# bacpop/sparrowhawk

Measured on AMD Instinct MI355X. Metric: Gbases/s assembled, k=31 150bp reads, higher is better.
Workload: dtype u64

## Files before the change

include/shk.h:

```cpp
#ifndef SHK_H
#define SHK_H

#include <stddef.h>
#include <stdint.h>

#ifdef __cplusplus
extern "C" {
#endif

#define SHK_OK 0
#define SHK_E_PARAM  (-1)
#define SHK_E_STATE  (-2)
#define SHK_E_PARSE  (-3)
#define SHK_E_OOM    (-4)
#define SHK_E_DEVICE (-5)
#define SHK_E_INTERNAL (-6)

#define SHK_HISTO_BINS 500
#define SHK_K_MIN 15
#define SHK_K_MAX 255

typedef struct shk_handle shk_handle;

typedef void (*shk_progress_cb)(const char *state, void *user);
// ... 66 lines not shown
void shk_packed_free(shk_packed *p);

uint32_t shk_key_words(shk_handle *h);
uint64_t shk_total_instances(shk_handle *h);
uint64_t shk_n_distinct(shk_handle *h);
int shk_get_distinct(shk_handle *h, uint64_t *keys, uint32_t *counts, uint64_t cap);
uint64_t shk_n_solid(shk_handle *h);
int shk_get_solid(shk_handle *h, uint64_t *keys, uint32_t *counts, uint64_t cap);
int shk_get_histo(shk_handle *h, uint64_t *histo500);
uint32_t shk_used_min_count(shk_handle *h);
int shk_get_adjacency(shk_handle *h, uint8_t *adj_initial, uint8_t *adj_final, uint8_t *alive,
                      uint64_t cap);
const char *shk_get_timings(shk_handle *h);
uint64_t shk_peak_device_bytes(shk_handle *h);
void shk_host_mem_counter(const int64_t *deltas, size_t n, uint64_t *peak, uint64_t *current);

int shk_host_canonical(const char *seq, uint32_t k, uint64_t *out_words , int *orient);
uint64_t shk_host_nthash(const char *seq, uint32_t k);
int shk_host_fit(const uint64_t *histo500, uint32_t *used_min_count);
char *shk_host_assembly_json(const char *seqs, const uint64_t *offsets, const uint64_t *kc, uint64_t n_contigs, uint32_t k);
char *shk_host_assembly_json_arriving(const char *seqs, const uint64_t *offsets, const uint64_t *kc, uint64_t n_contigs, uint32_t k,
                                      uint64_t piece_bytes, uint32_t delay_us);
void shk_host_free(void *p);
int shk_host_gunzip(const uint8_t *gz, size_t n, uint8_t **out, size_t *out_n, uint64_t *mt_members, double *reader_seconds);
int shk_device_gunzip(const uint8_t *gz, size_t n, uint8_t **out, size_t *out_n, const char **why, double *ms_total);
char *shk_host_unitig_assemble(uint32_t k, uint64_t n_recs, const uint64_t *first, const uint64_t *last, const uint64_t *len,
                               const uint64_t *kc, const uint8_t *circ, const uint64_t *min_key, const uint8_t *min_o,
                               const uint64_t *min_pos, int tips, int bubbles);
char *shk_device_unitig_assemble(uint32_t k, uint64_t n_recs, const uint64_t *first, const uint64_t *last, const uint64_t *len,
                                 const uint64_t *kc, const uint8_t *circ, const uint64_t *min_key, const uint8_t *min_o,
                                 const uint64_t *min_pos, int tips, int bubbles);

void shk_release_cached_memory(void);

int shk_measure_stream_read(size_t bytes, int iters, double *gbs);

const char *shk_version(void);

#ifdef __cplusplus
}
#endif
#endif
```

sparrowhawk_amd/_lib.py:

```python
import ctypes as C
import os

_HERE = os.path.dirname(os.path.abspath(__file__))
LIB_PATH = os.path.join(_HERE, "libshk_hip.so")

PROGRESS_CB = C.CFUNCTYPE(None, C.c_char_p, C.c_void_p)


class ShkPacked(C.Structure):
    _fields_ = [("bases", C.POINTER(C.c_uint32)), ("seg_off", C.POINTER(C.c_uint32)),
                ("n_seg", C.c_uint64), ("n_bases", C.c_uint64), ("n_reads", C.c_uint64),
                ("n_input_bases", C.c_uint64)]


_u64, _u32, _vp, _cp, _int, _sz = C.c_uint64, C.c_uint32, C.c_void_p, C.c_char_p, C.c_int, C.c_size_t
SIGNATURES = {
    "shk_new": (_vp, [_u32, _int, _u32, _u32, _u64, _int, _int, _int, _int]),
    "shk_new_error": (_int, []),
    "shk_new_error_message": (_cp, []),
    "shk_free": (None, [_vp]),
    "shk_last_error": (_cp, [_vp]),
    "shk_set_progress_cb": (None, [_vp, PROGRESS_CB, _vp]),
    "shk_preprocess": (_int, [_vp, _cp, _sz, _cp, _sz]),
    "shk_push_reads": (_int, [_vp, _cp, _sz]),
# ... 16 lines not shown
    "shk_comm_world": (_int, [_vp]),
    "shk_comm_free": (None, [_vp]),
    "shk_shard_preprocess": (_int, [_vp, _vp, _vp, _vp, _u64, _u64, _u64, _u32]),
    "shk_plan_exchange": (_int, [_vp, _u32, _u32, _u32, _vp, _vp, _vp, _vp, _vp]),
    "shk_choose_partitions": (_u32, [_u64, _u32, _u32]),
    "shk_plan_bgzf_windows": (C.c_int64, [_vp, _u64, _u64, _vp, _u64]),
    "shk_host_last_record_start": (_u64, [_cp, _sz]),
    "shk_device_last_record_start": (_int, [_cp, _sz, C.POINTER(_u64)]),
    "shk_pack_fastq": (_int, [_cp, _sz, _u32, _u32, C.POINTER(ShkPacked), C.POINTER(_cp)]),
    "shk_packed_free": (None, [C.POINTER(ShkPacked)]),
    "shk_key_words": (_u32, [_vp]),
    "shk_total_instances": (_u64, [_vp]),
    "shk_n_distinct": (_u64, [_vp]),
    "shk_get_distinct": (_int, [_vp, _vp, _vp, _u64]),
    "shk_n_solid": (_u64, [_vp]),
    "shk_get_solid": (_int, [_vp, _vp, _vp, _u64]),
    "shk_get_histo": (_int, [_vp, _vp]),
    "shk_used_min_count": (_u32, [_vp]),
    "shk_get_adjacency": (_int, [_vp, _vp, _vp, _vp, _u64]),
    "shk_get_timings": (_cp, [_vp]),
    "shk_peak_device_bytes": (_u64, [_vp]),
    "shk_host_mem_counter": (None, [_vp, _sz, C.POINTER(_u64), C.POINTER(_u64)]),
    "shk_host_canonical": (_int, [_cp, _u32, _vp, C.POINTER(_int)]),
    "shk_host_nthash": (_u64, [_cp, _u32]),
    "shk_host_fit": (_int, [_vp, C.POINTER(_u32)]),
    "shk_host_assembly_json": (_vp, [_cp, _vp, _vp, _u64, _u32]),
    "shk_host_assembly_json_arriving": (_vp, [_cp, _vp, _vp, _u64, _u32, _u64, _u32]),
    "shk_host_free": (None, [_vp]),
    "shk_host_gunzip": (_int, [_cp, _sz, C.POINTER(_vp), C.POINTER(_sz), C.POINTER(_u64), C.POINTER(C.c_double)]),
    "shk_device_gunzip": (_int, [_cp, _sz, C.POINTER(_vp), C.POINTER(_sz), C.POINTER(C.c_char_p), C.POINTER(C.c_double)]),
    "shk_host_unitig_assemble": (_vp, [_u32, _u64, _vp, _vp, _vp, _vp, _vp, _vp, _vp, _vp, _int, _int]),
    "shk_device_unitig_assemble": (_vp, [_u32, _u64, _vp, _vp, _vp, _vp, _vp, _vp, _vp, _vp, _int, _int]),
    "shk_release_cached_memory": (None, []),
    "shk_measure_stream_read": (_int, [_sz, _int, C.POINTER(C.c_double)]),
    "shk_version": (_cp, []),
}

_lib = None


def load():
    global _lib
    if _lib is None:
        if not os.path.exists(LIB_PATH):
            raise ImportError(
                f"{LIB_PATH} not found: build it with `python -c 'import __graft_entry__ as g; g.build()'` "
                "or `make -C sparrowhawk_amd/csrc` (there is no CPU fallback)")
        lib = C.CDLL(LIB_PATH, mode=C.RTLD_GLOBAL)
        for name, (res, args) in SIGNATURES.items():
            f = getattr(lib, name)
            f.restype, f.argtypes = res, args
        _lib = lib
    return _lib
```

sparrowhawk_amd/csrc/api.cpp:

```cpp
#include <atomic>
#include <stdio.h>
#include <stdlib.h>
#include <string.h>
#include <algorithm>
#include <mutex>
#include <new>
#include <set>
#include <string>
#include <thread>
#include <vector>

#include "fastq_gpu.h"
#include "inflate_gpu.h"
#include "inflate_mt.h"
#include "preprocess.h"
#include "unitig_graph.h"
#include "unitig_graph_gpu.h"

namespace shk { bool spectrum_fit(const uint64_t *histo500, uint32_t *out); }

using namespace shk;

static thread_local int g_new_err = 0;
static thread_local std::string g_new_msg;

enum class Poison { Never, AfterFirstBatch, Always };
template <typename F> static int guarded(shk_handle *h, Poison poison, F &&body) {
    if (!h) return SHK_E_PARAM;
    if (h->st == St::Failed) return fail(h, SHK_E_STATE, "the handle failed earlier (" + h->first_err + "): free it and start again");
    DevGuard g(h->pipe ? h->pipe->device() : current_device());
    MemGuard mg(h->mem);
    DeferScope park(h->pipe);
    int rc;
    try { rc = body(); }
    catch (const std::bad_alloc &) { rc = fail(h, SHK_E_OOM, "out of host memory"); }
    catch (const std::exception &e) { rc = fail(h, SHK_E_INTERNAL, std::string("unexpected exception: ") + e.what()); }
    catch (...) { rc = fail(h, SHK_E_INTERNAL, "unexpected exception"); }
    if (rc != SHK_OK && rc != SHK_E_STATE &&
        (poison == Poison::Always || (poison == Poison::AfterFirstBatch && (h->batches_started > 0 || h->st == St::Sharding))))
        { h->st = St::Failed; h->first_err = h->err; }
    return rc;
}

extern "C" {

static std::mutex g_live_mu;
static std::set<ShardComm *> &live_comms() { static auto *s = new std::set<ShardComm *>(); return *s; }
static bool comm_is_live(ShardComm *c) { std::lock_guard<std::mutex> lk(g_live_mu); return live_comms().count(c) != 0; }

void shk_release_cached_memory(void) { device_pool_trim(); big_trim(); }
int shk_measure_stream_read(size_t bytes, int iters, double *gbs) {
    std::string err;
    const int rc = stream_read_gbs(bytes, iters, gbs, err);
    return rc == 0 ? SHK_OK : code_of(Rc::Device, rc);
}

const char *shk_version(void) { return "sparrowhawk_amd 0.1 (gfx950)"; }
int shk_new_error(void) { return g_new_err; }
const char *shk_new_error_message(void) { return g_new_msg.c_str(); }

shk_handle *shk_new(uint32_t k, int verbose, uint32_t min_count, uint32_t min_qual, uint64_t chunk_size,
                    int do_bloom, int do_fit, int no_bubble_collapse, int no_dead_end_removal) {
    g_new_err = 0; g_new_msg.clear();
    if ((k & 1u) == 0 || k < SHK_K_MIN || k > SHK_K_MAX) {
        g_new_err = SHK_E_PARAM; g_new_msg = "k must be odd and within [15, 255]"; return nullptr;
    }
    if (min_qual > 93) { g_new_err = SHK_E_PARAM; g_new_msg = "min_qual out of range"; return nullptr; }
    if (min_count >= SHK_HISTO_BINS) { g_new_err = SHK_E_PARAM; g_new_msg = "min_count out of range"; return nullptr; }
    if (do_bloom && min_count < 3) {
        g_new_err = SHK_E_PARAM; g_new_msg = "Bloom mode requires min_count >= 3"; return nullptr;
    }
    shk_handle *h = new (std::nothrow) shk_handle();
    if (!h) { g_new_err = SHK_E_OOM; g_new_msg = "out of host memory"; return nullptr; }
    h->k = k; h->verbose = verbose != 0; h->min_count = min_count; h->min_qual = min_qual;
    h->chunk_size = chunk_size; h->do_bloom = do_bloom != 0; h->do_fit = do_fit != 0;
    h->no_bubble = no_bubble_collapse != 0; h->no_deadend = no_dead_end_removal != 0;
    std::string err;
    {
        MemGuard mg(h->mem);
        h->pipe = make_pipeline((int)k, err);
    }
    if (!h->pipe) { g_new_err = SHK_E_DEVICE; g_new_msg = err; delete h; return nullptr; }
    h->pipe->set_bloom(h->do_bloom);
// ... 750 lines not shown
```

sparrowhawk_amd/csrc/collapse.h:

```cpp
#pragma once

__device__ __forceinline__ bool node_sampled(uint32_t v, uint32_t split_mask) {
    return ((mix32(v ^ 0x5bd1e995u) >> 9) & split_mask) == 0;
}

template <int W> __device__ __forceinline__ unsigned long long km_prefix64(const KeyArr<W> &keys, uint32_t idx, int k) {
    const int used = 2 * k - 64 * (W - 1);
    const uint64_t hi = keys.w[W - 1][idx];
    if constexpr (W == 1) return hi;
    else return used >= 64 ? hi : ((hi << (64 - used)) | (keys.w[W - 2][idx] >> used));
}
template <int W> __device__ __forceinline__ bool node_key_less(const Graph<W> &g, uint32_t a, uint32_t b) {
    if ((a >> 1) == (b >> 1)) return a < b;
    const Kmer<W> ka = g.keys.load(a >> 1), kb = g.keys.load(b >> 1);
    if (km_less<W>(ka, kb)) return true;
    if (km_less<W>(kb, ka)) return false;
    return a < b;
}

struct FragRec { uint32_t next, len, last, chain_head ; unsigned long long sum; uint32_t owner, base; };
static_assert(sizeof(FragRec) == 32, "FragRec is one 32-byte record");
static constexpr int LF_THREADS = 1024, LF_ITEMS = 8;
static constexpr uint32_t LF_TILE = LF_THREADS * LF_ITEMS;
static constexpr uint16_t LF_STOP = 0xFFFFu, LF_DONE = 0xFFFEu;
// ... 165 lines not shown
                l_cnt[cur] = (j << 13) | pos;
                l_succ[cur] = LF_DONE;
                pos++;
                if (nx >= LF_TILE || pos >= LF_TILE) break;
                cur = nx;
            }
            const uint32_t v = base + j;
            FragRec f; f.next = winfo[base + cur].x; f.len = pos; f.last = base + cur; f.sum = sum; f.base = 0;
            const bool chain_head = winfo[v ^ 1u].x == NIL;
            f.chain_head = chain_head ? 1u : 0u;
            f.owner = (chain_head || node_sampled(v, split_mask)) ? ol[v].x : NIL;
            frag[v] = f;
        }
        __syncthreads();
#pragma unroll 2
        for (int it = 0; it < LF_ITEMS; it++) {
            const uint32_t j = (uint32_t)it * LF_THREADS + threadIdx.x;
            if (j >= size) break;
            uint2 o; o.x = NIL; o.y = 0;
            if (l_succ[j] == LF_DONE) { const uint32_t e = l_cnt[j]; o.x = base + (e >> 13); o.y = e & (LF_TILE - 1u); }
            ol[base + j] = o;
        }
        __syncthreads();
    }
}

struct SegRec { uint32_t node, next_spl, len, last; unsigned long long sum; uint32_t head, pad; };
static constexpr uint32_t HEAD_LINEAR = 1, HEAD_ORPHAN = 2;

template <int W>
__global__ __launch_bounds__(256) void k_walk_frags(const uint32_t *__restrict__ spl, const unsigned int *__restrict__ n_spl_p,
                                                    FragRec *__restrict__ frag, SegRec *__restrict__ segs,
                                                    uint32_t split_mask, unsigned long long *__restrict__ n_covered ,
                                                    uint32_t total , uint32_t *__restrict__ flags) {
    unsigned long long my_cov = 0;
    const uint32_t n_spl = *n_spl_p;
    for (uint32_t i = blockIdx.x * blockDim.x + threadIdx.x; i < n_spl; i += gridDim.x * blockDim.x) {
        const uint32_t s = spl[i];
        uint32_t cur = s, len = 0, nxt, last, is_head = 0;
        unsigned long long sum = 0;
        for (uint32_t hops = 0;; hops++) {
            const uint4 a = *reinterpret_cast<const uint4 *>(&frag[cur]);
            if (cur == s) is_head = a.w;
            const unsigned long long fs = frag[cur].sum;
            if (cur != s) { uint2 ob; ob.x = i; ob.y = len; *reinterpret_cast<uint2 *>(&frag[cur].owner) = ob; }
            sum += fs; len += a.y; last = a.z; nxt = a.x;
            if (last >= total || (nxt != NIL && nxt >= total) || hops >= total) { flags[0] = 1; last = s; nxt = NIL; break; }
            if (nxt == NIL || node_sampled(nxt, split_mask)) break;
            cur = nxt;
        }
        SegRec r; r.node = s; r.len = len; r.last = last; r.sum = sum; r.pad = 0;
        r.next_spl = (nxt == NIL) ? NIL : frag[nxt].owner;
        r.head = is_head ? HEAD_LINEAR : 0u;
        segs[i] = r;
        my_cov += len;
    }
    for (int o = 32; o > 0; o >>= 1) my_cov += __shfl_down(my_cov, o);
    if ((threadIdx.x & 63) == 0 && my_cov) atomicAdd(n_covered, my_cov);
}

static constexpr uint32_t ORPHAN_MAX = 1u << 16;
template <int W>
__global__ __launch_bounds__(256) void k_orphan_cycles(Graph<W> g, const uint8_t *__restrict__ alive,
                                                       const uint2 *__restrict__ winfo, uint2 *__restrict__ ol,
                                                       FragRec *__restrict__ frag,
                                                       uint32_t *__restrict__ spl, SegRec *__restrict__ segs,
                                                       unsigned int *__restrict__ n_spl,
                                                       uint32_t seg_cap, uint32_t *__restrict__ flags,
                                                       const unsigned long long *__restrict__ n_alive,
                                                       const unsigned long long *__restrict__ n_covered) {
    if (*n_alive == *n_covered || flags[0] == 4u) return;
    const uint32_t total = g.n * 2;
    for (uint32_t v = blockIdx.x * blockDim.x + threadIdx.x; v < total; v += gridDim.x * blockDim.x) {
        if (!alive[v >> 1]) continue;
        { uint32_t o_, p_; if (owner_of(ol, frag, v, o_, p_)) continue; }
        const uint2 w0 = winfo[v];
        uint32_t best = v, n = 1, cur = w0.x, last = v;
        unsigned long long sum = w0.y;
        bool ok = true;
        while (cur != v) {
            if (cur == NIL || n >= ORPHAN_MAX) { ok = false; break; }
            const uint2 w = winfo[cur];
            if (node_key_less<W>(g, cur, best)) best = cur;
            sum += w.y; n++; last = cur; cur = w.x;
        }
        if (!ok) { flags[0] = 1; continue; }
        if (best != v || (v & 1u)) continue;
        const uint32_t idx = atomicAdd(n_spl, 1u);
        if (idx >= seg_cap) { flags[0] = 2; atomicSub(n_spl, 1u); continue; }
        spl[idx] = v;
        cur = v;
        for (uint32_t j = 0; j < n; j++) {
            uint2 o; o.x = cur; o.y = 0; ol[cur] = o;
            uint2 ob; ob.x = idx; ob.y = j; *reinterpret_cast<uint2 *>(&frag[cur].owner) = ob;
            cur = winfo[cur].x;
        }
        SegRec r; r.node = v; r.next_spl = NIL; r.len = n; r.last = last; r.sum = sum; r.head = HEAD_ORPHAN; r.pad = 0;
        segs[idx] = r;
    }
}

struct RankRec { uint32_t P, A, m, d; unsigned long long K, dK; };
__global__ __launch_bounds__(256) void k_rank_init(const SegRec *__restrict__ segs, const unsigned int *__restrict__ n_spl_p,
                                                   RankRec *__restrict__ R) {
    const uint32_t n_spl = *n_spl_p;
    for (uint32_t s = blockIdx.x * blockDim.x + threadIdx.x; s < n_spl; s += gridDim.x * blockDim.x) {
        const SegRec r = segs[s];
        R[s].m = s; R[s].d = 0; R[s].dK = 0;
        if (r.head) { R[s].P = s; R[s].A = 0; R[s].K = 0; }
        if (r.next_spl != NIL && r.next_spl < n_spl) { R[r.next_spl].P = s; R[r.next_spl].A = r.len; R[r.next_spl].K = r.sum; }
    }
}
static constexpr int RANK_HOPS = 8;
__global__ __launch_bounds__(256) void k_rank_jump(const unsigned int *__restrict__ n_spl_p,
                                                   const RankRec *__restrict__ Ri, RankRec *__restrict__ Ro, uint32_t round = 0) {
    const uint32_t n_spl = *n_spl_p;
    {
        unsigned long long reach = 1; for (uint32_t r = 0; r < round; r++) reach *= RANK_HOPS;
        if (reach >= (unsigned long long)n_spl + 1ull) {
            for (uint32_t s = blockIdx.x * blockDim.x + threadIdx.x; s < n_spl; s += gridDim.x * blockDim.x) Ro[s] = Ri[s];
            return;
        }
    }
    for (uint32_t s = blockIdx.x * blockDim.x + threadIdx.x; s < n_spl; s += gridDim.x * blockDim.x) {
        uint32_t p = s, a = 0, bm = 0xFFFFFFFFu, bd = 0;
        unsigned long long kc = 0, bdk = 0;
#pragma unroll
        for (int h = 0; h < RANK_HOPS; h++) {
            const RankRec r = Ri[p];
            if (r.m < bm) { bm = r.m; bd = r.d + a; bdk = r.dK + kc; }
            a += r.A; kc += r.K;
            p = min(r.P, n_spl - 1u);
        }
        RankRec o; o.P = p; o.A = a; o.K = kc; o.m = bm; o.d = bd; o.dK = bdk;
        Ro[s] = o;
    }
}
struct HeadRec { uint32_t spl, head_node, tail_node, emit, rot, circ; unsigned long long len, kc; };
struct EmitRec { unsigned long long off; uint32_t rot, len; };
struct FinRec { uint32_t slot, base; };
struct RingMin { unsigned long long prefix; uint32_t vmin, is_ring; };
template <int W>
__global__ __launch_bounds__(256) void k_rank_tails(Graph<W> g, const SegRec *__restrict__ segs, const unsigned int *__restrict__ n_spl_p,
                                                    const RankRec *__restrict__ R,
                                                    HeadRec *__restrict__ heads, uint32_t *__restrict__ slot_of,
                                                    RingMin *__restrict__ ringmin,
                                                    unsigned int *__restrict__ n_heads, unsigned int *__restrict__ n_cyc) {
    __shared__ uint32_t blk_cyc;
    if (threadIdx.x == 0) blk_cyc = 0;
    __syncthreads();
    const uint32_t n_spl = *n_spl_p;
    uint32_t my_cyc = 0;
    for (uint32_t s = blockIdx.x * blockDim.x + threadIdx.x; s < n_spl; s += gridDim.x * blockDim.x) {
        const SegRec r = segs[s];
        const RankRec me = R[s];
        const uint32_t hd = segs[me.P].head;
        if (hd != 0u) {
            if (r.next_spl != NIL) continue;
            const uint32_t root = me.P;
            const uint32_t slot = atomicAdd(n_heads, 1u);
            HeadRec h; h.spl = root; h.head_node = segs[root].node; h.tail_node = r.last; h.rot = 0;
            h.len = (unsigned long long)me.A + r.len; h.kc = me.K + r.sum;
            if (hd == HEAD_ORPHAN) { h.circ = 1; h.emit = 1; }
            else {
                h.circ = 0;
                const Kmer<W> a = g.seq(h.head_node), b = g.seq(h.tail_node ^ 1u);
                if (km_less<W>(a, b)) h.emit = 1;
                else if (km_less<W>(b, a)) h.emit = 0;
                else h.emit = h.head_node <= (h.tail_node ^ 1u);
            }
            heads[slot] = h; slot_of[root] = slot;
            RingMin rm; rm.prefix = ~0ull; rm.vmin = NIL; rm.is_ring = 0; ringmin[slot] = rm;
        } else {
            my_cyc++;
            if (r.next_spl != me.m) continue;
            const uint32_t root = me.m;
            const uint32_t slot = atomicAdd(n_heads, 1u);
            HeadRec h; h.spl = root; h.head_node = segs[root].node; h.tail_node = r.last; h.circ = 1;
            h.len = (unsigned long long)me.d + r.len; h.kc = me.dK + r.sum;
            h.emit = 0; h.rot = 0;
            heads[slot] = h; slot_of[root] = slot;
            RingMin rm; rm.prefix = ~0ull; rm.vmin = NIL; rm.is_ring = 1; ringmin[slot] = rm;
        }
    }
    if (my_cyc) atomicAdd(&blk_cyc, my_cyc);
    __syncthreads();
    if (threadIdx.x == 0 && blk_cyc) atomicAdd(n_cyc, blk_cyc);
}
__global__ __launch_bounds__(256) void k_rank_fin(const SegRec *__restrict__ segs, const unsigned int *__restrict__ n_spl_p,
                                                  const RankRec *__restrict__ R, const uint32_t *__restrict__ slot_of,
                                                  FinRec *__restrict__ fin) {
    const uint32_t n_spl = *n_spl_p;
    for (uint32_t s = blockIdx.x * blockDim.x + threadIdx.x; s < n_spl; s += gridDim.x * blockDim.x) {
        const RankRec me = R[s];
        const bool ring = segs[me.P].head == 0u;
        FinRec f; f.slot = slot_of[ring ? me.m : me.P]; f.base = ring ? me.d : me.A;
        fin[s] = f;
    }
}

__global__ __launch_bounds__(LF_THREADS) void k_tile_final(uint32_t n_rows, const uint32_t *__restrict__ row_starts, uint32_t tile_rows,
                                                           uint2 *__restrict__ ol, const FragRec *__restrict__ frag,
                                                           const FinRec *__restrict__ fin,
                                                           const unsigned long long *__restrict__ skip = nullptr ,
                                                           const uint32_t *__restrict__ flags = nullptr ) {
    if (skip && (skip[0] | skip[1])) return;
    if (flags && flags[0] == 4u) return;
    __shared__ uint2 l_chain[LF_TILE];
    __shared__ uint32_t t_lo, t_hi;
    tile_bounds(row_starts, n_rows, tile_rows, &t_lo, &t_hi);
    __syncthreads();
    const uint32_t hi = t_hi;
    for (uint32_t c = t_lo; c < hi; c += LF_TILE / 2u) {
        const uint32_t base = 2u * c;
        const uint32_t size = 2u * (min(c + LF_TILE / 2u, hi) - c);
        uint2 t[LF_ITEMS];
#pragma unroll
        for (int it = 0; it < LF_ITEMS; it++) {
            const uint32_t j = (uint32_t)it * LF_THREADS + threadIdx.x;
            const uint32_t v = base + j;
            t[it].x = NIL; t[it].y = 0;
            if (j < size) {
                t[it] = ol[v];
                if (t[it].x == v) {
// ... 224 lines not shown
```

sparrowhawk_amd/csrc/count_part.h:

```cpp
#pragma once
#include <hip/hip_runtime.h>
#include <stdint.h>
#include <type_traits>
#include "kmer.h"

namespace shk {

static constexpr int PART_THREADS = 1024;
static constexpr int COUNT_THREADS = 1024;
static constexpr int PART_MAX_P = 16384;

struct PartParams {
    uint32_t P, G, slice_cap;
    int k, m;
    uint32_t max_n;
};

template <int RW> struct Rec { uint64_t w[RW]; };

__device__ __forceinline__ uint64_t sel4(uint32_t b, uint64_t t0, uint64_t t1, uint64_t t2, uint64_t t3) {
    uint64_t lo = (b & 1) ? t1 : t0;
    uint64_t hi = (b & 1) ? t3 : t2;
    return (b & 2) ? hi : lo;
}
// ... 581 lines not shown
        for (uint32_t b = threadIdx.x; b < 500; b += COUNT_THREADS)
            if (ctl.histo[b]) atomicAdd(&histo[b], (unsigned long long)ctl.histo[b]);
    }
    if (!n_emit) return;
    __syncthreads();
    const unsigned long long gbase = ((unsigned long long)ctl.emit_base_hi << 32) | ctl.emit_base_lo;
    for (uint32_t i = threadIdx.x; i < n_emit; i += COUNT_THREADS) {
        const uint32_t sl = list[i];
        const unsigned long long o = gbase + i;
        if (o < out_cap) {
            Kmer<W> x;
            if constexpr (W == 1) x.w[0] = tb.key0[sl];
            else {
#pragma unroll
                for (int j = 0; j < W; j++) x.w[j] = tb.key[j][sl];
            }
            out_keys.store(o, x);
            out_cnt[o] = tb.cnt[sl];
        }
    }
}

struct OvfRec { uint32_t p, est_distinct; unsigned long long instances; };
struct OvfItem { uint32_t p, F, cap, pad; unsigned long long base; };
static constexpr uint32_t OVF_MAX_F = 256;

struct RunView {
    const unsigned long long *run_addr16;
    const uint32_t *run_cnt;
    uint32_t S;
    int k;
    const uint32_t *weights = nullptr;
    unsigned long long rec_base16 = 0;
};

__global__ __launch_bounds__(256) void k_make_runs(const uint32_t *__restrict__ fill, PartParams pp,
                                                   const uint64_t *recs, uint32_t rec_words,
                                                   unsigned long long *__restrict__ run_addr16,
                                                   uint32_t *__restrict__ run_cnt) {
    const uint64_t n = (uint64_t)pp.P * pp.G;
    const unsigned long long base16 = (unsigned long long)recs >> 4;
    for (uint64_t i = (uint64_t)blockIdx.x * blockDim.x + threadIdx.x; i < n; i += (uint64_t)gridDim.x * blockDim.x) {
        run_addr16[i] = base16 + i * pp.slice_cap * (rec_words / 2u);
        run_cnt[i] = min(fill[i], pp.slice_cap);
    }
}

__global__ __launch_bounds__(256) void k_part_totals(const uint32_t *__restrict__ fill, PartParams pp,
                                                     unsigned long long *__restrict__ totals) {
    const uint32_t p = blockIdx.x;
    unsigned long long t = 0;
    for (uint32_t g = threadIdx.x; g < pp.G; g += blockDim.x) t += min(fill[(uint64_t)p * pp.G + g], pp.slice_cap);
    for (int o = 32; o > 0; o >>= 1) t += __shfl_down(t, o);
    __shared__ unsigned long long part[4];
    if ((threadIdx.x & 63) == 0) part[threadIdx.x >> 6] = t;
    __syncthreads();
    if (threadIdx.x == 0) totals[p] = part[0] + part[1] + part[2] + part[3];
}

template <int RW>
__global__ __launch_bounds__(256) void k_pack_partition(const uint64_t *__restrict__ recs,
                                                        const uint32_t *__restrict__ fill, PartParams pp,
                                                        const unsigned long long *__restrict__ base,
                                                        uint64_t *__restrict__ dst) {
    __shared__ uint32_t pre[257];
    const uint32_t p = blockIdx.x;
    const int lane = threadIdx.x & 63;
    if (threadIdx.x < 64) {
        uint32_t run = 0;
        for (uint32_t g0 = 0; g0 < pp.G; g0 += 64) {
            const uint32_t g = g0 + threadIdx.x;
            const uint32_t f = g < pp.G ? min(fill[(uint64_t)p * pp.G + g], pp.slice_cap) : 0u;
            uint32_t incl = f;
            for (int o = 1; o < 64; o <<= 1) { uint32_t v = __shfl_up(incl, o); if (lane >= o) incl += v; }
            if (g < pp.G) pre[g] = run + incl - f;
            run += __shfl(incl, 63);
        }
        if (threadIdx.x == 0) pre[pp.G] = run;
    }
    __syncthreads();
    const uint32_t R = pre[pp.G];
    const uint64_t *src_p = recs + (uint64_t)p * pp.G * pp.slice_cap * RW;
    uint64_t *dst_p = dst + base[p] * RW;
    for (uint32_t r = threadIdx.x; r < R; r += blockDim.x) {
        uint32_t lo = 0, hi = pp.G;
        while (hi - lo > 1) { const uint32_t mid = (lo + hi) >> 1; if (pre[mid] <= r) lo = mid; else hi = mid; }
        const uint64_t *src = src_p + ((uint64_t)lo * pp.slice_cap + (r - pre[lo])) * RW;
#pragma unroll
        for (int o = 0; o < RW; o += 2)
            *reinterpret_cast<ulonglong2 *>(dst_p + (uint64_t)r * RW + o) = *reinterpret_cast<const ulonglong2 *>(src + o);
    }
}

template <int RW>
__global__ __launch_bounds__(256) void k_merge_runs(RunView rvw, const unsigned long long *__restrict__ base,
                                                    uint64_t *__restrict__ dst) {
    __shared__ uint32_t pre[257];
    __shared__ unsigned long long roff[256];
    const uint32_t p = blockIdx.x, S_runs = rvw.S;
    const int lane = threadIdx.x & 63;
    if (threadIdx.x < 64) {
        uint32_t run = 0;
        for (uint32_t g0 = 0; g0 < S_runs; g0 += 64) {
            const uint32_t g = g0 + threadIdx.x;
            const uint32_t f = g < S_runs ? rvw.run_cnt[(uint64_t)p * S_runs + g] : 0u;
            if (g < S_runs) roff[g] = rvw.run_addr16[(uint64_t)p * S_runs + g];
            uint32_t incl = f;
            for (int o = 1; o < 64; o <<= 1) { const uint32_t v = __shfl_up(incl, o); if (lane >= o) incl += v; }
            if (g < S_runs) pre[g] = run + incl - f;
            run += __shfl(incl, 63);
        }
        if (threadIdx.x == 0) pre[S_runs] = run;
    }
    __syncthreads();
    const uint32_t R = pre[S_runs];
    uint64_t *dst_p = dst + base[p] * RW;
    for (uint32_t r = threadIdx.x; r < R; r += blockDim.x) {
        uint32_t lo = 0, hi = S_runs;
        while (hi - lo > 1) { const uint32_t mid = (lo + hi) >> 1; if (pre[mid] <= r) lo = mid; else hi = mid; }
        const uint64_t *src = reinterpret_cast<const uint64_t *>(roff[lo] << 4) + (uint64_t)(r - pre[lo]) * RW;
#pragma unroll
        for (int o = 0; o < RW; o += 2)
            *reinterpret_cast<ulonglong2 *>(dst_p + (uint64_t)r * RW + o) = *reinterpret_cast<const ulonglong2 *>(src + o);
    }
}

template <int W, bool WEIGHTED = false >
__global__ __launch_bounds__(COUNT_THREADS) void k_count_partitions(
    RunView rvw, uint32_t n_parts, uint32_t threshold,
    unsigned long long *__restrict__ histo, KeyArr<W> out_keys, uint32_t *__restrict__ out_cnt,
    unsigned long long out_cap, unsigned long long *__restrict__ out_cursor,
    unsigned long long *__restrict__ n_inst, uint32_t *__restrict__ flags,
    const uint32_t *__restrict__ part_list ,
    OvfRec *__restrict__ ovf ,
    uint32_t *__restrict__ ovf_n,
    uint32_t *__restrict__ work_counter ,
    uint32_t probe_blocks, uint32_t defer_after ) {
    constexpr int RW = 2 * W;
    constexpr uint32_t S = CountShared<W>::S;
    __shared__ CountShared<W> tb;
    __shared__ CountCtl ctl;
    __shared__ uint32_t whist[500];
    __shared__ uint32_t wtot[4];
    const int lane = threadIdx.x & 63;
    const int k = rvw.k;
    const uint32_t S_runs = rvw.S;
    for (uint32_t b = threadIdx.x; b < 500; b += COUNT_THREADS) whist[b] = 0;
    if (threadIdx.x == 0) ctl.n_inst = 0;
    auto load_runs = [&](uint32_t pi, uint32_t &cnt, unsigned long long &addr) {
        cnt = 0; addr = 0;
        if (pi < n_parts && threadIdx.x < S_runs) {
            const uint32_t pp = part_list ? part_list[pi] : pi;
            cnt = rvw.run_cnt[(uint64_t)pp * S_runs + threadIdx.x];
            addr = rvw.run_addr16[(uint64_t)pp * S_runs + threadIdx.x];
        }
    };
    uint32_t nx_cnt; unsigned long long nx_addr;
    load_runs(blockIdx.x, nx_cnt, nx_addr);
  uint32_t pi_next = 0;
  for (uint32_t pi = blockIdx.x; pi < n_parts; pi = pi_next) {
    const uint32_t p = part_list ? part_list[pi] : pi;
    if (threadIdx.x == 0) ctl.next_pi = gridDim.x + atomicAdd(work_counter, 1u);
    {
        const uint32_t f = nx_cnt;
        uint32_t incl = f;
        if (threadIdx.x < 256) {
            for (int o = 1; o < 64; o <<= 1) { const uint32_t v = __shfl_up(incl, o); if (lane >= o) incl += v; }
            if (lane == 63) wtot[threadIdx.x >> 6] = incl;
        }
        __syncthreads();
        if (threadIdx.x < 256) {
            uint32_t off = 0;
            for (uint32_t w = 0; w < (threadIdx.x >> 6); w++) off += wtot[w];
            if (threadIdx.x < S_runs) { ctl.pre[threadIdx.x] = off + incl - f; ctl.roff[threadIdx.x] = nx_addr; }
        }
        if (threadIdx.x == 0) {
            ctl.pre[S_runs] = wtot[0] + wtot[1] + wtot[2] + wtot[3];
            ctl.sp = 1; ctl.st_res[0] = 0; ctl.st_step[0] = 1; ctl.st_factor[0] = 1; ctl.st_next[0] = 0;
            ctl.part_inst = 0; ctl.n_used = 0;
            uint32_t force = 0;
            if (ovf && defer_after && pi >= probe_blocks) {
                const uint32_t x = __hip_atomic_load(&ovf_n[1], __ATOMIC_RELAXED, __HIP_MEMORY_SCOPE_AGENT);
                const uint32_t n_over = x >> 16, n_tried = x & 0xFFFFu;
                force = (n_over >= defer_after && 4u * n_over >= 3u * n_tried) ? 1u : 0u;
            }
            ctl.overflow = force;
        }
// ... 153 lines not shown
        }
        if (over) {
            if (mod >= 4096 || ctl.sp + 1 > 16) { if (threadIdx.x == 0) flags[0] = 1; break; }
            __syncthreads();
            if (threadIdx.x == 0) {
                const uint32_t num = ctl.prog_num ? ctl.prog_num : ctl.prog_den;
                const double est = (double)ctl.n_used * (double)ctl.prog_den / (double)num;
                uint32_t factor = 2;
                while ((double)factor * (0.6 * S) < est && mod * factor < 4096u) factor <<= 1;
                ctl.st_res[ctl.sp] = res; ctl.st_step[ctl.sp] = mod; ctl.st_factor[ctl.sp] = factor; ctl.st_next[ctl.sp] = 0;
                ctl.sp += 1;
            }
            continue;
        }
        static_assert(2u * decltype(tb.rt)::SR >= S, "emit list");
        table_emit<W>(tb, ctl, mine, threshold, histo, out_keys, out_cnt, out_cap, out_cursor, reinterpret_cast<uint16_t *>(tb.rt.rst), whist);
    }
    if (threadIdx.x == 0 && ovf && defer_after) atomicAdd(&ovf_n[1], 1u);
   }();
  }
    __syncthreads();
    for (uint32_t b = threadIdx.x; b < 500; b += COUNT_THREADS)
        if (whist[b]) atomicAdd(&histo[b], (unsigned long long)whist[b]);
    if (threadIdx.x == 0 && ctl.n_inst) atomicAdd(n_inst, ctl.n_inst);
}


template <int W> struct DedupeShared {
    RecTable<W, (W == 1 ? 3072u : ((69632u / (16u * W + 6u)) & ~63u))> rt;
};
template <int W>
__global__ __launch_bounds__(COUNT_THREADS, W <= 2 ? 8 : 4) void k_dedupe_partitions(
                                                                     RunView rvw, uint32_t p_first, uint32_t n_parts,
                                                                     const unsigned long long *__restrict__ base,
                                                                     uint64_t *__restrict__ out_recs, uint32_t *__restrict__ out_w,
                                                                     uint32_t *__restrict__ n_out, uint32_t *__restrict__ work_counter,
                                                                     OvfRec *__restrict__ ovf , uint32_t *__restrict__ ovf_n,
                                                                     uint32_t defer_after, uint32_t kmer_cap,
                                                                     uint32_t *__restrict__ verdict_out ) {
    constexpr int RW = 2 * W;
    __shared__ DedupeShared<W> tb;
    __shared__ CountCtl ctl;
    __shared__ uint32_t wtot[4];
    constexpr uint32_t SR = decltype(tb.rt)::SR;
    const int lane = threadIdx.x & 63;
    const int k = rvw.k;
    const uint32_t S_runs = rvw.S;
    const uint32_t n_here = n_parts - p_first;
    __shared__ uint32_t forced_sh;
    if (threadIdx.x == 0) forced_sh = 0;
    __syncthreads();
    bool forced = false;
    uint32_t pi_next = 0;
    for (uint32_t pi = blockIdx.x; pi < n_here; pi = pi_next) {
        const uint32_t p = p_first + pi;
        uint32_t f = 0; unsigned long long addr = 0;
        if (threadIdx.x < S_runs) { f = rvw.run_cnt[(uint64_t)p * S_runs + threadIdx.x]; addr = rvw.run_addr16[(uint64_t)p * S_runs + threadIdx.x]; }
        forced = forced_sh != 0;
        if (forced) {
            unsigned long long inst = 0;
            const uint64_t *src = reinterpret_cast<const uint64_t *>(addr << 4);
            for (uint32_t i = 0; i < f; i++) inst += (src[(uint64_t)i * RW + RW - 1] >> 58) + 1ull;
            __syncthreads();
            if (threadIdx.x == 0) { ctl.part_inst = 0; ctl.next_pi = gridDim.x + atomicAdd(work_counter, 1u); }
            __syncthreads();
            for (int o = 32; o > 0; o >>= 1) inst += __shfl_down(inst, o);
            if (lane == 0 && inst) atomicAdd(&ctl.part_inst, inst);
            __syncthreads();
            pi_next = ctl.next_pi;
            if (threadIdx.x == 0) {
                n_out[p] = 0;
                if (ctl.part_inst) { const uint32_t slot = atomicAdd(ovf_n, 1u); OvfRec o; o.p = p; o.est_distinct = 0u; o.instances = ctl.part_inst; ovf[slot] = o; }
            }
            continue;
        }
        uint32_t incl = f;
        if (threadIdx.x < 256) {
            for (int o = 1; o < 64; o <<= 1) { const uint32_t v = __shfl_up(incl, o); if (lane >= o) incl += v; }
            if (lane == 63) wtot[threadIdx.x >> 6] = incl;
        }
        __syncthreads();
        if (threadIdx.x < 256) {
            uint32_t off = 0;
            for (uint32_t w = 0; w < (threadIdx.x >> 6); w++) off += wtot[w];
            if (threadIdx.x < S_runs) { ctl.pre[threadIdx.x] = off + incl - f; ctl.roff[threadIdx.x] = addr; }
        }
        if (threadIdx.x == 0) {
            ctl.pre[S_runs] = wtot[0] + wtot[1] + wtot[2] + wtot[3];
            ctl.rec_used = 0; ctl.n_emit = 0; ctl.part_inst = 0;
            ctl.next_pi = gridDim.x + atomicAdd(work_counter, 1u);
// ... 78 lines not shown
            for (int o = 1; o < 64; o <<= 1) { const uint32_t u = __shfl_up(incl2, o); if (lane >= o) incl2 += u; }
            rt.nbase[threadIdx.x] = n_pass + incl2 - v;
            if (threadIdx.x == 63) ctl.n_recs = n_pass + incl2;
        }
        __syncthreads();
        const bool hand = ovf && (ctl.n_recs > kmer_cap || (R > kmer_cap / 4u && 2u * ctl.n_recs > R));
        if (ovf && threadIdx.x == 0 && R) {
            const uint32_t add = hand ? 0x10001u : 1u;
            const uint32_t x = atomicAdd(&ovf_n[1], add) + add;
            const uint32_t n_over = x >> 16, n_tried = x & 0xFFFFu;
            if (defer_after && n_over >= defer_after && 2u * n_over >= n_tried) {
                forced_sh = 1u;
                if (verdict_out) atomicOr(verdict_out, 0x80000000u);
            }
        }
        if (hand) { hand_over(); continue; }
        for (uint32_t s = threadIdx.x; s < SR; s += COUNT_THREADS) {
            const uint32_t st = rt.rst[s];
            if (st < 3u) continue;
            const uint32_t at = atomicAdd(&rt.nbase[(uint32_t)(rt.w[s][RW - 1] >> 58)], 1u);
            uint64_t r[RW];
#pragma unroll
            for (int o = 0; o < RW; o++) r[o] = rt.w[s][o];
            part_store_record<RW>(r, dst + (uint64_t)at * RW);
            dst_w[at] = st - 2u;
        }
        __syncthreads();
        if (threadIdx.x == 0) n_out[p] = ctl.n_recs;
    }
}

template <int W>
__global__ __launch_bounds__(COUNT_THREADS, W <= 2 ? 8 : 4) void k_count_weighted(
    const uint64_t *__restrict__ recs, const uint32_t *__restrict__ weights, const unsigned long long *__restrict__ base,
    const uint32_t *__restrict__ n_recs, uint32_t p_first, uint32_t n_parts, uint32_t merge , int k, uint32_t threshold,
    unsigned long long *__restrict__ histo, KeyArr<W> out_keys, uint32_t *__restrict__ out_cnt,
    unsigned long long out_cap, unsigned long long *__restrict__ out_cursor,
    unsigned long long *__restrict__ n_inst, OvfRec *__restrict__ ovf, uint32_t *__restrict__ ovf_n,
    unsigned long long *__restrict__ work_and_tally ,
    uint32_t probe_groups, uint32_t defer_after,
    EmitRanges er ) {
    constexpr int RW = 2 * W;
    constexpr uint32_t S = KmerTable<W>::S;
    __shared__ KmerTable<W> tb;
    __shared__ CountCtlCore ctl;
    constexpr uint32_t ELIST = W == 1 ? S : 64;
    __shared__ uint16_t elist[ELIST];
    __shared__ uint32_t whist[500];
    __shared__ uint32_t next_g_sh, force_sh;
    const int lane = threadIdx.x & 63;
    for (uint32_t b = threadIdx.x; b < 500; b += COUNT_THREADS) whist[b] = 0;
    if (threadIdx.x == 0) ctl.n_inst = 0;
    const uint32_t n_groups = (n_parts + merge - 1) / merge;
    unsigned long long mine = 0;
    auto count_range = [&](const uint32_t (&pm)[4], uint32_t nm) -> bool {
        uint32_t Rj[4]; unsigned long long bj[4]; uint32_t Rt = 0;
#pragma unroll
        for (int j = 0; j < 4; j++) {
            const bool in = (uint32_t)j < nm;
            Rj[j] = in ? n_recs[pm[j]] : 0u; bj[j] = in ? base[pm[j]] : 0ull;
            Rt += Rj[j];
        }
        auto fetch = [&](uint32_t r, Rec<RW> &rec, uint32_t &wgt) {
            if (r < Rt) {
                unsigned long long at = bj[0] + r;
                uint32_t pre = Rj[0];
#pragma unroll
// ... 139 lines not shown
    uint64_t *dp = dst + dst_base[p] * RW;
    for (uint32_t r = threadIdx.x; r < R; r += blockDim.x) {
#pragma unroll
        for (int o = 0; o < RW; o += 2)
            *reinterpret_cast<ulonglong2 *>(dp + (uint64_t)r * RW + o) = *reinterpret_cast<const ulonglong2 *>(sp + (uint64_t)r * RW + o);
        dst_w[dst_base[p] + r] = src_w[src_base[p] + r];
    }
}

static constexpr uint32_t BLOOM_WORDS = 24576;
template <int W, bool BLOOM>
__global__ __launch_bounds__(COUNT_THREADS) void k_ovf_scatter(RunView rvw, const OvfItem *__restrict__ items,
                                                               uint64_t *__restrict__ kmers,
                                                               uint32_t *__restrict__ bucket_fill,
                                                               uint32_t *__restrict__ new_count) {
    constexpr int RW = 2 * W;
    __shared__ uint32_t pre[257];
    __shared__ uint32_t cursor[OVF_MAX_F];
    __shared__ uint32_t bloom[BLOOM ? BLOOM_WORDS : 1];
    __shared__ uint32_t n_new;
    if constexpr (BLOOM) {
        for (uint32_t i = threadIdx.x; i < BLOOM_WORDS; i += COUNT_THREADS) bloom[i] = 0;
        if (threadIdx.x == 0) n_new = 0;
    }
    uint32_t my_new = 0;
    const OvfItem it = items[blockIdx.x];
    const uint32_t p = it.p, S_runs = rvw.S;
    const int lane = threadIdx.x & 63;
    const int k = rvw.k;
    if (threadIdx.x < 64) {
        uint32_t run = 0;
        for (uint32_t g0 = 0; g0 < S_runs; g0 += 64) {
            const uint32_t g = g0 + threadIdx.x;
            uint32_t f = g < S_runs ? rvw.run_cnt[(uint64_t)p * S_runs + g] : 0u;
            uint32_t incl = f;
            for (int o = 1; o < 64; o <<= 1) { uint32_t v = __shfl_up(incl, o); if (lane >= o) incl += v; }
            if (g < S_runs) pre[g] = run + incl - f;
            run += __shfl(incl, 63);
        }
        if (threadIdx.x == 0) pre[S_runs] = run;
    }
    for (uint32_t b = threadIdx.x; b < OVF_MAX_F; b += COUNT_THREADS) cursor[b] = 0;
    __syncthreads();
    const uint32_t R = pre[S_runs];
    const uint32_t F = it.F;
    for (uint32_t r = threadIdx.x; r < R; r += COUNT_THREADS) {
        uint32_t lo = 0, hi = S_runs;
        while (hi - lo > 1) { const uint32_t mid = (lo + hi) >> 1; if (pre[mid] <= r) lo = mid; else hi = mid; }
        const uint64_t *src = reinterpret_cast<const uint64_t *>(rvw.run_addr16[(uint64_t)p * S_runs + lo] << 4) + (uint64_t)(r - pre[lo]) * RW;
        Rec<RW> rec;
#pragma unroll
        for (int o = 0; o < RW; o += 2) {
            const ulonglong2 v2 = *reinterpret_cast<const ulonglong2 *>(src + o);
            rec.w[o] = v2.x; rec.w[o + 1] = v2.y;
        }
        const uint32_t n = (uint32_t)(rec.w[RW - 1] >> 58) + 1u;
        Kmer<W> f = km_zero<W>();
        for (uint32_t s = 0; s < n; s++) {
            if (s) {
#pragma unroll
                for (int o = 0; o < RW - 1; o++) rec.w[o] = (rec.w[o] >> 2) | (rec.w[o + 1] << 62);
                rec.w[RW - 1] >>= 2;
            }
            Kmer<W> rv;
#pragma unroll
            for (int j = 0; j < W; j++) rv.w[j] = ~rec.w[j];
            rv.w[W - 1] &= km_topmask<W>(k);
            if (s) km_push_back<W>(f, (uint32_t)(rec.w[W - 1] >> ((2 * (k - 1)) & 63)) & 3u, k);
            else f = km_revcomp<W>(rv, k);
            const bool use_r = km_less<W>(rv, f);
            Kmer<W> c;
#pragma unroll
            for (int j = 0; j < W; j++) c.w[j] = use_r ? rv.w[j] : f.w[j];
            const uint32_t hk = km_mix32<W>(c);
            if constexpr (BLOOM) {
                const uint32_t h2 = mix32(hk ^ 0xC2B2AE35u);
                const uint32_t word = (uint32_t)(((uint64_t)h2 * BLOOM_WORDS) >> 32);
                const uint32_t b0 = hk & 31u, b1 = (hk >> 5) & 31u;
                const uint32_t bits = (1u << b0) | (1u << (b1 == b0 ? (b0 + 1u) & 31u : b1));
                const uint32_t old = atomicOr(&bloom[word], bits);
                if ((old & bits) != bits) { my_new++; continue; }
            }
// ... 194 lines not shown
```

sparrowhawk_amd/csrc/graph_part.h:

```cpp
#pragma once

struct MinScan {
    Nt32State first, last;
    uint32_t h_first, h_last;
    uint32_t min_wo_first;
    uint32_t min_wo_last;
    __device__ __forceinline__ uint32_t min_all() const { return min(min_wo_first, h_first); }
};

template <int W> __device__ __forceinline__ uint32_t km_base(const Kmer<W> &x, int k, int j) {
    return km_bits2<W>(x, 2 * (k - 1 - j));
}

template <int W> __device__ __forceinline__ MinScan km_min_scan(const Kmer<W> &x, int k, int gm) {
    MinScan r;
    Nt32State nt{0, 0};
    for (int j = 0; j < gm; j++) nt32_init_step(nt, km_base<W>(x, k, j), (unsigned)j);
    r.first = nt; r.h_first = nt32_canonical(nt);
    r.min_wo_first = 0xFFFFFFFFu; r.min_wo_last = r.h_first;
    const int w = k - gm + 1;
    uint32_t h = r.h_first;
    for (int q = 1; q < w; q++) {
        nt32_roll(nt, km_base<W>(x, k, q - 1), km_base<W>(x, k, q + gm - 1), (unsigned)gm);
        h = nt32_canonical(nt);
// ... 602 lines not shown
        tips[t] = r;
    }
}

template <int W>
__global__ __launch_bounds__(256) void k_tip_decide(Graph<W> g, const TipRec *__restrict__ tips,
                                                    const unsigned int *__restrict__ n_tips_p,
                                                    const uint32_t *__restrict__ tip_head,
                                                    uint8_t *__restrict__ kill) {
    const uint32_t n_tips = *n_tips_p;
    for (uint32_t a = blockIdx.x * blockDim.x + threadIdx.x; a < n_tips; a += gridDim.x * blockDim.x) {
        const TipRec me = tips[a];
        const uint32_t d = g.indeg(me.junction);
        uint32_t t = 0; bool best = true;
        const Kmer<W> myfirst = g.keys.load(me.start >> 1);
        for (uint32_t b = tip_head[me.junction]; b != NIL; b = tips[b].next) {
            t++;
            if (b == a) continue;
            const TipRec o = tips[b];
            bool better;
            if (o.len != me.len) better = o.len > me.len;
            else if (o.sum != me.sum) better = o.sum > me.sum;
            else better = km_less<W>(g.keys.load(o.start >> 1), myfirst);
            if (better) best = false;
        }
        kill[a] = (t < d) ? 1 : (best ? 0 : 1);
    }
}

template <int W>
__global__ __launch_bounds__(256) void k_tip_remove(Graph<W> g, const TipRec *__restrict__ tips,
                                                    const unsigned int *__restrict__ n_tips_p, const uint8_t *__restrict__ kill,
                                                    uint32_t *__restrict__ tip_head,
                                                    uint8_t *__restrict__ mark) {
    const uint32_t n_tips = *n_tips_p;
    for (uint32_t a = blockIdx.x * blockDim.x + threadIdx.x; a < n_tips; a += gridDim.x * blockDim.x) {
        const TipRec me = tips[a];
        if (kill[a]) {
            uint32_t cur = me.start;
            for (uint32_t i = 0; i < me.len; i++) {
                mark[cur >> 1] = 1;
                if (i + 1 < me.len) cur = g.only_out(cur);
            }
        }
    }
}

__global__ __launch_bounds__(256) void k_tip_reset_heads(const TipRec *__restrict__ tips, const unsigned int *__restrict__ n_tips_p,
                                                         uint32_t *__restrict__ tip_head) {
    const uint32_t n_tips = *n_tips_p;
    for (uint32_t a = blockIdx.x * blockDim.x + threadIdx.x; a < n_tips; a += gridDim.x * blockDim.x)
        tip_head[tips[a].junction] = NIL;
}

template <int W>
__global__ __launch_bounds__(256) void k_fork_candidates(Graph<W> g, const uint8_t *__restrict__ alive,
                                                         uint32_t *__restrict__ cand,
                                                         unsigned int *__restrict__ n_cand) {
    const int lane = threadIdx.x & 63;
    const uint32_t stride = gridDim.x * blockDim.x;
    const uint32_t n_round = (g.n + stride - 1) / stride * stride;
    for (uint32_t i = blockIdx.x * blockDim.x + threadIdx.x; i < n_round; i += stride) {
        uint32_t a = 0; bool al = false;
        if (i < g.n) { a = g.adj[i]; al = alive[i] != 0; }
#pragma unroll
        for (uint32_t o = 0; o < 2; o++) {
            const bool p = al && __popc(outmask_of(a, o)) >= 2;
            const unsigned long long m = __ballot(p);
            if (!m) continue;
            unsigned int base = 0;
            if (lane == 0) base = atomicAdd(n_cand, (unsigned int)__popcll(m));
            base = __shfl(base, 0);
            if (p) cand[base + __popcll(m & ((1ull << lane) - 1ull))] = 2u * i + o;
        }
    }
}

template <int W>
__global__ __launch_bounds__(256) void k_bubble(Graph<W> g, const uint32_t *__restrict__ cand,
                                                const unsigned int *__restrict__ n_cand_p, uint8_t *__restrict__ mark) {
    const uint32_t T_BUB = 2u * (uint32_t)g.k;
    const uint32_t n_cand = *n_cand_p;
    for (uint32_t c = blockIdx.x * blockDim.x + threadIdx.x; c < n_cand; c += gridDim.x * blockDim.x) {
        const uint32_t S = cand[c];
        const uint32_t om = g.outmask(S);
        uint32_t first[4], end[4], len[4];
        unsigned long long sum[4];
        bool ok[4];
#pragma unroll
        for (uint32_t b = 0; b < 4; b++) {
            ok[b] = false; first[b] = NIL; end[b] = NIL; len[b] = 0; sum[b] = 0;
            if (!((om >> b) & 1u)) continue;
            const uint32_t bn = g.follow(S, b);
            if (bn == NIL || g.indeg(bn) != 1) continue;
            first[b] = bn;
            uint32_t cur = bn, l = 1;
            unsigned long long s = g.cnt[bn >> 1];
            for (;;) {
                if (g.outdeg(cur) != 1) break;
                const uint32_t n = g.only_out(cur);
                if (n == NIL) break;
                if (g.indeg(n) >= 2) { end[b] = n; ok[b] = true; break; }
                if (l + 1 > T_BUB) break;
                l++; s += g.cnt[n >> 1]; cur = n;
            }
            len[b] = l; sum[b] = s;
        }
#pragma unroll
        for (uint32_t a = 0; a < 4; a++) {
            if (!ok[a]) continue;
            const uint32_t E = end[a];
            {
                const Kmer<W> ks = g.keys.load(S >> 1), ke = g.keys.load(E >> 1);
                bool le;
                if (km_less<W>(ks, ke)) le = true;
                else if (km_less<W>(ke, ks)) le = false;
                else le = (S & 1u) <= ((E ^ 1u) & 1u);
                if (!le) continue;
            }
            uint32_t grp = 0; bool best = true;
            const Kmer<W> fa = g.keys.load(first[a] >> 1);
#pragma unroll
            for (uint32_t b = 0; b < 4; b++) {
                if (!ok[b] || end[b] != E) continue;
                grp++;
                if (b == a) continue;
                const unsigned long long l = sum[b] * len[a], r = sum[a] * len[b];
                bool better;
                if (l != r) better = l > r;
                else if (len[b] != len[a]) better = len[b] < len[a];
                else better = km_less<W>(g.keys.load(first[b] >> 1), fa);
                if (better) best = false;
            }
            if (grp >= 2 && !best) {
                uint32_t cur = first[a];
                for (uint32_t i = 0; i < len[a]; i++) {
                    mark[cur >> 1] = 1;
                    if (i + 1 < len[a]) cur = g.only_out(cur);
                }
            }
        }
    }
}

__global__ __launch_bounds__(256) void k_collect_marked(uint32_t n, uint8_t *__restrict__ mark,
                                                        uint8_t *__restrict__ alive,
                                                        uint32_t *__restrict__ removed,
                                                        unsigned int *__restrict__ n_removed) {
    const int lane = threadIdx.x & 63;
    const uint32_t stride = gridDim.x * blockDim.x;
    const uint32_t n_round = (n + stride - 1) / stride * stride;
    for (uint32_t i = blockIdx.x * blockDim.x + threadIdx.x; i < n_round; i += stride) {
        bool p = false;
        if (i < n && mark[i]) { mark[i] = 0; if (alive[i]) { alive[i] = 0; p = true; } }
        const unsigned long long m = __ballot(p);
        if (!m) continue;
        unsigned int base = 0;
        if (lane == 0) base = atomicAdd(n_removed, (unsigned int)__popcll(m));
        base = __shfl(base, 0);
        if (p) removed[base + __popcll(m & ((1ull << lane) - 1ull))] = i;
    }
}

__device__ __forceinline__ void adj_clear_bit(uint8_t *adj, uint32_t idx, uint32_t bit) {
    uint32_t *wptr = (uint32_t *)adj + (idx >> 2);
    atomicAnd(wptr, ~((1u << bit) << (8 * (idx & 3u))));
}
// ... 30 lines not shown
```

sparrowhawk_amd/csrc/pipeline.h:

```cpp
#pragma once
#include <stdint.h>
#include <string>
#include <vector>
#include <map>
#include <memory>

namespace shk {

struct ShardComm;

class TextArrival {
public:
    virtual ~TextArrival() {}
    virtual const char *base() const = 0;
    virtual size_t total() const = 0;
    virtual void wait_range(size_t begin, size_t end) = 0;
    void wait_all() { wait_range(0, total()); }
    virtual int finish(std::string &err) = 0;
};

struct RawContig {
    const char *ext = nullptr; size_t ext_n = 0;
    std::string own;
    uint64_t kc = 0;
// ... 22 lines not shown
    virtual void set_verbose(bool on) = 0;
    virtual void single_batch_resident(bool on) = 0;
    virtual int histogram(uint64_t histo[500], uint32_t emit_threshold, std::string &err) = 0;
    virtual int filter(uint32_t threshold, std::string &err) = 0;
    virtual uint64_t total_instances() const = 0;
    virtual uint64_t n_distinct() const = 0;
    virtual uint64_t n_solid() const = 0;
    virtual int get_distinct(uint64_t *keys, uint32_t *counts, uint64_t cap, std::string &err) = 0;
    virtual int get_solid(uint64_t *keys, uint32_t *counts, uint64_t cap, std::string &err) = 0;
    virtual int build_graph(std::string &err) = 0;
    virtual int correct(bool tips, bool bubbles, std::string &err) = 0;
    virtual int collapse(std::vector<RawContig> &out, std::string &err, const char **json = nullptr, size_t *json_len = nullptr,
                         uint64_t *n_contigs = nullptr, TextArrival **arrival = nullptr) = 0;
    virtual int get_adjacency(uint8_t *adj_initial, uint8_t *adj_final, uint8_t *alive,
                              uint64_t cap, std::string &err) = 0;
    virtual int shard_partition(const uint32_t *d_bases, const uint32_t *d_seg_off, uint64_t n_seg, uint64_t n_bases,
                                uint32_t n_partitions, std::vector<uint64_t> &part_records, std::string &err) = 0;
    virtual uint32_t rec_words() const = 0;
    virtual int shard_pack(void *d_send, const uint64_t *base_records, uint32_t n_partitions, std::string &err) = 0;
    virtual int shard_dedupe(std::vector<uint64_t> &part_records, std::string &err) = 0;
    virtual int shard_pack_dedup(void *d_send, void *d_send_w, const uint64_t *base_records, uint32_t n_partitions, std::string &err) = 0;
    virtual void shard_drop_dedup() = 0;
    virtual int shard_count(const void *d_recv, const void *d_recv_w , const uint64_t *run_off, const uint32_t *run_cnt,
                            uint32_t n_owned, uint32_t n_sources, uint32_t emit_threshold, uint64_t histo[500], std::string &err) = 0;
    virtual int shard_rows(uint32_t threshold, const void **keys_soa, const void **cnt, uint64_t *n, std::string &err) = 0;
    virtual int shard_set_solid(const void *const *keys_soa, const void *cnt, uint64_t n, const uint64_t histo[500],
                                uint64_t total_instances, std::string &err) = 0;
    virtual int shard_keep_local(uint32_t world, uint32_t rank, uint32_t n_count_partitions, const uint64_t *rows_per_rank,
                                 const uint64_t histo[500], uint64_t total_instances, std::string &err) = 0;
    virtual bool sharded_graph() const = 0;
    virtual uint64_t n_solid_global() const = 0;
    virtual int shard_assemble(ShardComm *comm, bool tips, bool bubbles, std::vector<RawContig> &out, std::string &err) = 0;
    virtual StageTimes &times() = 0;
    virtual void drain() = 0;
    virtual void *stream() = 0;
    virtual int device() const = 0;
};

class DeferScope {
public:
    explicit DeferScope(IPipeline *pipe);
    ~DeferScope();
    DeferScope(const DeferScope &) = delete;
    DeferScope &operator=(const DeferScope &) = delete;
private:
    IPipeline *pipe_; void *list_; void *prev_;
};

IPipeline *make_pipeline(int k, std::string &err);
int device_count();
int current_device();
int set_device(int dev);

int host_canonical(const char *seq, uint32_t k, uint64_t *out_words, int *orient);
uint64_t host_nthash(const char *seq, uint32_t k);

int device_upload(const void *host, size_t bytes, void **dptr, std::string &err);
void device_free(void *dptr);
void device_pool_trim();
void *device_pool_alloc(size_t &bytes);
int stream_read_gbs(size_t bytes, int iters, double *gbs, std::string &err);
void device_pool_release(void *p, size_t bytes);
std::shared_ptr<void> mem_acct_new();
std::shared_ptr<void> mem_acct_set(std::shared_ptr<void> a);
uint64_t mem_acct_peak(const std::shared_ptr<void> &a);
uint64_t mem_acct_current(const std::shared_ptr<void> &a);
void mem_acct_replay(const int64_t *deltas, size_t n, uint64_t *peak, uint64_t *current);
int device_stream_sync(void *stream, std::string &err);
int device_copy_h2d_async(void *dst, const void *src, size_t bytes, void *stream, std::string &err);
int device_download(void *host, const void *dptr, size_t bytes, std::string &err);

}
```

sparrowhawk_amd/csrc/pipeline.hip:

```cpp
#include <hip/hip_runtime.h>
#include <hipcub/hipcub.hpp>
#include <thread>
#include <stdint.h>
#include <stdio.h>
#include <stdlib.h>
#include <string.h>
#include <algorithm>
#include <atomic>
#include <chrono>
#include <map>
#include <memory>
#include <mutex>
#include <string>
#include <vector>

#include "kmer.h"
#include "pipeline.h"
#include "shard_comm.h"
#include "unitig_graph.h"
#include "unitig_graph_gpu.h"

namespace shk {

#define HIPCHK(call)                                                                      \
    do {                                                                                  \
        hipError_t _e = (call);                                                           \
        if (_e != hipSuccess) {                                                           \
            err = std::string(#call) + ": " + hipGetErrorString(_e);                      \
            return -5;                                                                    \
        }                                                                                 \
    } while (0)
#define WAIT_STREAM()                                                                     \
    do {                                                                                  \
        n_host_waits_++;                                                                  \
        if (wd_comm_) { if (int _rc = comm_stream_wait(wd_comm_, stream_, err)) return _rc; } \
        else HIPCHK(stream_wait(stream_));                                                \
    } while (0)

static constexpr uint32_t NIL = 0xFFFFFFFFu;
static constexpr int CTL_WORDS = 32;
static constexpr int CTL_ER = 22;
static constexpr uint32_t GP_MAX = 131072;
static constexpr uint64_t EMPTY64 = ~0ull;
static constexpr int MAX_PROBE = 4096;
static constexpr uint64_t UNITIG_DEVICE_MIN_DEFAULT = 65536;
static constexpr int SPLIT_LOG_DEFAULT = 6;

template <int W> struct KeyArr {
    uint64_t *w[W];
    __device__ __forceinline__ Kmer<W> load(uint64_t i) const {
        Kmer<W> x;
#pragma unroll
        for (int j = 0; j < W; j++) x.w[j] = w[j][i];
        return x;
    }
    __device__ __forceinline__ void store(uint64_t i, const Kmer<W> &x) const {
#pragma unroll
        for (int j = 0; j < W; j++) w[j][i] = x.w[j];
    }
};

template <int W> struct CountTable {
    KeyArr<W> keys;
    uint32_t *cnt;
    uint32_t *state;
    uint64_t mask;
};

struct GraphTable {
    uint64_t *e;
    uint2 *scan = nullptr;
    uint32_t scan_n = 0;
    uint8_t *occ;
// ... 140 lines not shown
DeferScope::DeferScope(IPipeline *pipe) : pipe_(pipe) {
    auto *v = new (std::nothrow) std::vector<std::pair<void *, size_t>>();
    if (v) { try { v->reserve(256); } catch (...) {} }
    list_ = v; prev_ = tls_defer; tls_defer = v;
}
DeferScope::~DeferScope() {
    auto *v = (std::vector<std::pair<void *, size_t>> *)list_;
    tls_defer = (std::vector<std::pair<void *, size_t>> *)prev_;
    if (!v) return;
    if (!v->empty()) {
        if (pipe_) pipe_->drain();
        else (void)hipDeviceSynchronize();
        for (auto &b : *v) dev_pool().put(b.first, b.second);
    }
    delete v;
}

static std::mutex g_stream_mu;
static std::multimap<int, hipStream_t> &stream_cache() { static auto *c = new std::multimap<int, hipStream_t>(); return *c; }
static hipStream_t stream_pool_get(int dev) {
    std::lock_guard<std::mutex> lk(g_stream_mu);
    auto it = stream_cache().find(dev);
    if (it == stream_cache().end()) return nullptr;
    hipStream_t s = it->second; stream_cache().erase(it); return s;
}
static void stream_pool_put(int dev, hipStream_t s) {
    {
        std::lock_guard<std::mutex> lk(g_stream_mu);
        if (stream_cache().size() < 32) { stream_cache().emplace(dev, s); return; }
    }
    (void)hipStreamDestroy(s);
}

static std::mutex &upload_token(int dev) { static std::mutex m[16]; return m[(unsigned)dev % 16u]; }

static inline int grid_for(uint64_t work, int block = 256, int max_blocks = 256 * 16) {
    uint64_t b = (work + block - 1) / block;
    if (b < 1) b = 1;
    if (b > (uint64_t)max_blocks) b = max_blocks;
    return (int)b;
}

static inline hipError_t stream_wait(hipStream_t s) {
    static const bool blocking = getenv("SHK_BLOCKING_SYNC") != nullptr;
    if (blocking) return hipStreamSynchronize(s);
    const auto t0 = std::chrono::steady_clock::now();
    for (;;) {
        const hipError_t e = hipStreamQuery(s);
        if (e != hipErrorNotReady) return e;
        if (std::chrono::steady_clock::now() - t0 > std::chrono::milliseconds(5)) return hipStreamSynchronize(s);
    }
}

struct EvTimer {
    hipEvent_t a, b; hipStream_t st; bool ok = false;
    explicit EvTimer(hipStream_t s, bool on = true) : st(s) {
        if (!on) return;
        ok = hipEventCreate(&a) == hipSuccess && hipEventCreate(&b) == hipSuccess;
        if (ok) (void)hipEventRecord(a, st);
    }
    bool on() const { return ok; }
    double stop() {
        if (!ok) return 0.0;
        (void)hipEventRecord(b, st); (void)hipEventSynchronize(b);
        float ms = 0; (void)hipEventElapsedTime(&ms, a, b);
        return ms;
// ... 4 lines not shown
        if (!ok) return 0.0;
        (void)hipEventSynchronize(b);
        float ms = 0; (void)hipEventElapsedTime(&ms, a, b);
        return ms;
    }
    struct Pending { std::string name; hipEvent_t a, b; };
    void stop_later(const char *name, std::vector<Pending> &pending) {
        if (!ok) return;
        (void)hipEventRecord(b, st);
        pending.push_back(Pending{name, a, b});
        ok = false;
    }
    static void resolve(std::vector<Pending> &pending, StageTimes &times) {
        for (auto &p : pending) {
            (void)hipEventSynchronize(p.b);
            float ms = 0; (void)hipEventElapsedTime(&ms, p.a, p.b);
            times.add(p.name, ms);
            (void)hipEventDestroy(p.a); (void)hipEventDestroy(p.b);
        }
        pending.clear();
    }
};

static inline uint64_t env_u64(const char *name, uint64_t dflt) {
    const char *v = getenv(name);
    return (v && *v) ? strtoull(v, nullptr, 10) : dflt;
}

__global__ __launch_bounds__(256) void k_fill2(uint32_t *a, unsigned long long na, uint32_t va, uint32_t *b, unsigned long long nb, uint32_t vb) {
    const unsigned long long stride = (unsigned long long)gridDim.x * blockDim.x;
    for (unsigned long long i = (unsigned long long)blockIdx.x * blockDim.x + threadIdx.x; i < na + nb; i += stride) {
        if (i < na) a[i] = va; else b[i - na] = vb;
    }
}
__global__ __launch_bounds__(256) void k_stride_fill(unsigned long long *out, uint32_t n, unsigned long long stride) {
    for (uint32_t i = blockIdx.x * blockDim.x + threadIdx.x; i < n; i += gridDim.x * blockDim.x) out[i] = (unsigned long long)i * stride;
}
static inline hipError_t fill2_async(void *a, size_t bytes_a, uint32_t va, void *b, size_t bytes_b, uint32_t vb, hipStream_t st) {
    const unsigned long long na = bytes_a / 4, nb = bytes_b / 4;
    const unsigned long long blocks = std::min<unsigned long long>((na + nb + 255) / 256, 2048ull);
    if (!blocks) return hipSuccess;
    hipLaunchKernelGGL(k_fill2, dim3((uint32_t)blocks), dim3(256), 0, st, (uint32_t *)a, na, va, (uint32_t *)b, nb, vb);
    return hipGetLastError();
}

static constexpr uint32_t ARRIVAL_SLAB = 64u << 10;
__global__ __launch_bounds__(256) void k_text_to_host(const char *__restrict__ src, char *__restrict__ dst_host, unsigned long long bytes,
                                                      uint32_t n_slabs, uint32_t *__restrict__ flags_host) {
    for (uint32_t s = blockIdx.x; s < n_slabs; s += gridDim.x) {
        const unsigned long long o = (unsigned long long)s * ARRIVAL_SLAB;
        const uint32_t m = (uint32_t)(bytes - o < ARRIVAL_SLAB ? bytes - o : ARRIVAL_SLAB);
        const uint4 *a = reinterpret_cast<const uint4 *>(src + o);
        uint4 *d = reinterpret_cast<uint4 *>(dst_host + o);
        const uint32_t nv = m >> 4;
#pragma unroll 4
        for (uint32_t i = threadIdx.x; i < nv; i += 256) d[i] = a[i];
        if (threadIdx.x < (m & 15u)) dst_host[o + (nv << 4) + threadIdx.x] = src[o + (nv << 4) + threadIdx.x];
        __threadfence_system();
        __syncthreads();
        if (threadIdx.x == 0) __hip_atomic_store(&flags_host[s], 1u, __ATOMIC_RELEASE, __HIP_MEMORY_SCOPE_SYSTEM);
    }
}
__global__ __launch_bounds__(1024) void k_ends_to_host(const char *__restrict__ text, const unsigned long long *__restrict__ src ,
                                                       uint32_t nc, uint32_t E, char *__restrict__ ends_host, uint32_t *__restrict__ flag_host) {
    const unsigned long long total = (unsigned long long)nc * 2ull * E;
    for (unsigned long long t = threadIdx.x; t < total; t += blockDim.x) {
        const uint32_t c = (uint32_t)(t / (2ull * E)), r = (uint32_t)(t % (2ull * E)), side = r / E, j = r % E;
        const unsigned long long off = src[2 * c], len = src[2 * c + 1];
        const unsigned long long m = len < E ? len : (unsigned long long)E;
// ... 31 lines not shown
        }
    }
    void wait_range(size_t begin, size_t end) override {
        if (end > total_) end = total_;
        if (begin >= end) return;
        for (size_t s = begin / ARRIVAL_SLAB; s <= (end - 1) / ARRIVAL_SLAB; s++) if (!spin_until(flags_ + s, failed_)) return;
    }
    int finish(std::string &err) override {
        const hipError_t e = hipStreamSynchronize(st_);
        if (e != hipSuccess || failed_.load()) { err = std::string("download of the contigs failed") + (e != hipSuccess ? std::string(": ") + hipGetErrorString(e) : std::string()); return -5; }
        return 0;
    }
    std::atomic<bool> failed_{false};
private:
    char *base_ = nullptr; size_t total_ = 0; volatile uint32_t *flags_ = nullptr; uint32_t n_slabs_ = 0; hipStream_t st_ = nullptr;
};

static inline int part_win(int k) {
    static const int forced = [] { const char *e = getenv("SHK_PART_WIN"); return e ? atoi(e) : 0; }();
    if (k < 23) return 8;
    if (k < 31) return 16;
    if (forced == 16 || forced == 18 || forced == 20) return forced;
    return k <= 32 ? 18 : 16;
}
static inline int part_m(int k) { return k - part_win(k) + 1; }

template <int W> class Pipeline : public IPipeline {
public:
    explicit Pipeline(int k) : k_(k) {}
    ~Pipeline() override {
        drain();
        EvTimer::resolve(pending_timers_, times_);
        if (copy_stream_) { (void)hipStreamSynchronize(copy_stream_); stream_pool_put(stream_dev_ + 1000, copy_stream_); }
        if (stream_) stream_pool_put(stream_dev_, stream_);
    }
    int init(std::string &err) {
        HIPCHK(hipGetDevice(&stream_dev_));
        { int cus = 0; (void)hipDeviceGetAttribute(&cus, hipDeviceAttributeMultiprocessorCount, stream_dev_); n_cus_ = cus > 0 ? cus : 256; }
        stream_ = stream_pool_get(stream_dev_);
        if (!stream_) HIPCHK(hipStreamCreate(&stream_));
        HIPCHK(ctl_.alloc(CTL_WORDS, err) ? hipErrorOutOfMemory : hipSuccess);
        if (mbox_.alloc(MBOX_BYTES, err)) return -4;
        return 0;
    }
    StageTimes &times() override { EvTimer::resolve(pending_timers_, times_); return times_; }
    void drain() override {
        if (copy_stream_) (void)hipStreamSynchronize(copy_stream_);
        if (!stream_) return;
        std::string e;
        if (wd_comm_) (void)comm_stream_wait(wd_comm_, stream_, e);
        else (void)hipStreamSynchronize(stream_);
    }
    void *stream() override { return (void *)stream_; }
    int device() const override { return stream_dev_; }
    uint64_t total_instances() const override { return total_instances_; }
    uint64_t n_distinct() const override { return n_distinct_; }
    uint64_t n_solid() const override { return n_solid_; }

    int alloc_table(uint64_t slots, std::string &err) {
        for (int j = 0; j < W; j++) if (int rc = tkeys_[j].alloc(slots, err)) return rc;
        if (int rc = tcnt_.alloc(slots, err)) return rc;
        if (W > 1) if (int rc = tstate_.alloc(slots, err)) return rc;
        tslots_ = slots;
        if (W == 1) HIPCHK(hipMemsetAsync(tkeys_[0].p, 0xFF, slots * 8, stream_));
        else HIPCHK(hipMemsetAsync(tstate_.p, 0, slots * 4, stream_));
        HIPCHK(hipMemsetAsync(tcnt_.p, 0, slots * 4, stream_));
        return 0;
    }
    CountTable<W> table_view() {
        CountTable<W> t;
        for (int j = 0; j < W; j++) t.keys.w[j] = tkeys_[j].p;
        t.cnt = tcnt_.p; t.state = tstate_.p; t.mask = tslots_ - 1;
        return t;
    }

    int count_batch_global(const uint32_t *d_bases, const uint32_t *d_seg_off, uint64_t n_seg,
                           uint64_t n_bases, std::string &err) {
        if (n_seg >= 0xFFFFFFFFull || n_bases >= 0xFFFFFFFFull) { err = "batch too large (>= 2^32 bases)"; return -1; }
        if (n_seg == 0) return 0;
        const uint64_t inst_ub = n_bases - n_seg * (uint64_t)(k_ - 1);
        if (tslots_ == 0) {
            uint64_t want = inst_ub / 4 + 1024;
            uint64_t slots = 1ull << 16;
            while (slots < want) slots <<= 1;
            if (int rc = alloc_table(slots, err)) return rc;
            pending_.clear();
        }
        pending_.push_back({d_bases, d_seg_off, n_seg});
        for (;;) {
            HIPCHK(hipMemsetAsync(ctl_.p, 0, CTL_WORDS * sizeof(unsigned long long), stream_));
            EvTimer t(stream_);
            hipLaunchKernelGGL(k_count_segments<W>, dim3(grid_for(n_seg)), dim3(256), 0, stream_, d_bases,
                               d_seg_off, (uint32_t)n_seg, k_, table_view(), (uint32_t *)(ctl_.p + 1),
                               ctl_.p + 0);
            HIPCHK(hipGetLastError());
            double ms = t.stop();
            unsigned long long h[2];
            HIPCHK(hipMemcpyAsync(h, ctl_.p, sizeof h, hipMemcpyDeviceToHost, stream_));
            WAIT_STREAM();
            if ((uint32_t)h[1] == 0) {
                times_.add("count_kernel", ms);
                total_instances_ += h[0];
                return 0;
            }
            if (pending_.size() > 1) { err = "count table overflow across batches"; return -6; }
            times_.add("count_retry", ms);
            if (int rc = alloc_table(tslots_ * 4, err)) return rc;
        }
    }

    template <int WBLK, int NBLK>
    void launch_partition_t(const uint32_t *d_bases, const uint32_t *d_seg_off, uint32_t n_seg) {
        hipLaunchKernelGGL((k_partition<W, WBLK, NBLK>), dim3(pp_.G), dim3(PART_THREADS), 0, stream_, d_bases, d_seg_off,
                           n_seg, pp_, recs_.p, fill_.p, (uint32_t *)(ctl_.p + 8));
    }
    void launch_partition(int win, const uint32_t *d_bases, const uint32_t *d_seg_off, uint32_t n_seg) {
        if (win == 20) launch_partition_t<10, 2>(d_bases, d_seg_off, n_seg);
        else if (win == 18) launch_partition_t<9, 2>(d_bases, d_seg_off, n_seg);
        else if (win == 16) launch_partition_t<16, 1>(d_bases, d_seg_off, n_seg);
        else launch_partition_t<8, 1>(d_bases, d_seg_off, n_seg);
    }

    int count_batch(const uint32_t *d_bases, const uint32_t *d_seg_off, uint64_t n_seg, uint64_t n_bases,
                    std::string &err) override {
        return count_batch_impl(d_bases, d_seg_off, nullptr, nullptr, n_seg, n_bases, err);
    }
    int count_batch_host(uint32_t *d_bases, uint32_t *d_seg_off, const uint32_t *h_bases, const uint32_t *h_seg_off,
                         uint64_t n_seg, uint64_t n_bases, std::string &err) override {
        return count_batch_impl(d_bases, d_seg_off, h_bases, h_seg_off, n_seg, n_bases, err);
    }
    int count_batch_pieces(const DevPiece *pieces, size_t n_pieces, std::string &err) override {
        std::vector<DevPiece> list;
        uint64_t n_seg = 0, n_bases = 0;
        for (size_t i = 0; i < n_pieces; i++)
            if (pieces[i].n_seg) { list.push_back(pieces[i]); n_seg += pieces[i].n_seg; n_bases += pieces[i].n_bases; }
        if (list.empty()) return 0;
        if (list.size() == 1) return count_batch_impl(list[0].d_bases, list[0].d_seg_off, nullptr, nullptr, n_seg, n_bases, err);
        if (global_mode_) {
            for (const DevPiece &pc : list)
                if (int rc = count_batch_impl(pc.d_bases, pc.d_seg_off, nullptr, nullptr, pc.n_seg, pc.n_bases, err)) return rc;
            return 0;
        }
        piece_list_ = std::move(list);
        struct Clear { std::vector<DevPiece> &v; ~Clear() { v.clear(); } } clear{piece_list_};
        return count_batch_impl(piece_list_[0].d_bases, piece_list_[0].d_seg_off, nullptr, nullptr, n_seg, n_bases, err);
    }
    void launch_partition_all(int wblk, const uint32_t *d_bases, const uint32_t *d_seg_off, uint64_t n_seg) {
// ... 8 lines not shown
            h_bases = nullptr;
        }
        if (global_mode_) return count_batch_global(d_bases, d_seg_off, n_seg, n_bases, err);
        if (n_seg >= 0xFFFFFFFFull || n_bases >= 0xFFFFFFFFull) { err = "batch too large (>= 2^32 bases)"; return -1; }
        if (n_seg == 0) return 0;
        if (have_parts_) if (int rc = pack_current_batch(err)) return rc;
        constexpr int RW = 2 * W;
        const int wblk = part_win(k_);
        const uint64_t inst_ub = n_bases - n_seg * (uint64_t)(k_ - 1);
        const int cus = n_cus_;
        const uint64_t n_super = (n_seg + PART_THREADS - 1) / PART_THREADS;
        pp_.k = k_; pp_.m = k_ - wblk + 1;
        pp_.max_n = std::min<uint32_t>(32u * RW - 3u - (uint32_t)(k_ - 1), 63u);
        if (uint64_t mn = env_u64("SHK_PART_MAXN", 0)) pp_.max_n = std::min<uint32_t>(pp_.max_n, (uint32_t)mn);
        pp_.G = (uint32_t)std::min<uint64_t>((uint64_t)std::min(cus, 256), n_super);
        if (uint64_t fg = env_u64("SHK_PART_G", 0)) pp_.G = (uint32_t)std::min<uint64_t>(pp_.G, fg);
        uint32_t P = 64;
        const uint64_t per_part = env_u64("SHK_PART_INST", W == 1 ? 100000 : 40000);
        while (P < (uint32_t)PART_MAX_P && (uint64_t)P * per_part < inst_ub) P <<= 1;
        if (uint64_t fp = env_u64("SHK_PART_P", 0)) P = (uint32_t)fp;
        if (forced_P_) P = forced_P_;
        if (!batches_.empty()) P = pp_.P;
        pp_.P = P;
        const uint64_t per_rec = pp_.max_n >= 16 ? 4 : 2;
        uint64_t cap = inst_ub / (per_rec * P * pp_.G) + 32 + env_u64("SHK_SLICE_PAD", 0);
        if (cap_override_) { cap = cap_override_; cap_override_ = 0; }
        for (int attempt = 0; attempt < 2; attempt++) {
            if (env_u64("SHK_SLICE_NOSKEW", 0) == 0)
                while ((cap * RW * 8) % 2048 < 256 || (cap * RW * 8) % 2048 > 1792) cap++;
            if (cap * pp_.G > 0xFFFFFFF0ull) { err = "a partition would hold more than 2^32 records"; return -1; }
            pp_.slice_cap = (uint32_t)cap;
            const uint64_t n_slices = (uint64_t)P * pp_.G;
            if (int rc = recs_.alloc(n_slices * cap * RW, err)) return rc;
            if (int rc = fill_.alloc(n_slices, err)) return rc;
            HIPCHK(fill2_async(fill_.p, n_slices * 4, 0u, ctl_.p, CTL_WORDS * sizeof(unsigned long long), 0u, stream_));
            EvTimer t(stream_);
            if (h_bases && attempt == 0) {
                uint64_t C = env_u64("SHK_H2D_PIECES", 4);
                if (C < 1) C = 1;
                while (C > 1 && n_seg / C < (uint64_t)PART_THREADS * pp_.G) C--;
                if (!copy_stream_) copy_stream_ = stream_pool_get(stream_dev_ + 1000);
                if (!copy_stream_) HIPCHK(hipStreamCreateWithFlags(&copy_stream_, hipStreamNonBlocking));
                const uint64_t n_words = (n_bases + 15) / 16 + 1;
                std::vector<hipEvent_t> evs((size_t)C, nullptr);
                struct EvGuard { std::vector<hipEvent_t> &v; ~EvGuard() { for (auto e : v) if (e) (void)hipEventDestroy(e); } } evg{evs};
                struct CopyDrain { hipStream_t s; std::unique_lock<std::mutex> token; ~CopyDrain() { (void)hipStreamSynchronize(s); } }
                    copy_drain{copy_stream_, std::unique_lock<std::mutex>(upload_token(stream_dev_))};
                for (uint64_t c = 0; c < C; c++) {
                    const uint64_t s0 = n_seg * c / C, s1 = n_seg * (c + 1) / C;
                    const uint64_t w0 = h_seg_off[s0] >> 4, w1 = std::min<uint64_t>(n_words, (((uint64_t)h_seg_off[s1] + 15) >> 4) + 1);
                    HIPCHK(hipMemcpyAsync((void *)(d_seg_off + s0), h_seg_off + s0, (s1 - s0 + 1) * 4, hipMemcpyHostToDevice, copy_stream_));
                    HIPCHK(hipMemcpyAsync((void *)(d_bases + w0), h_bases + w0, (w1 - w0) * 4, hipMemcpyHostToDevice, copy_stream_));
                    HIPCHK(hipEventCreateWithFlags(&evs[c], hipEventDisableTiming));
                    HIPCHK(hipEventRecord(evs[c], copy_stream_));
                    HIPCHK(hipStreamWaitEvent(stream_, evs[c], 0));
                    launch_partition(wblk, d_bases, d_seg_off + s0, (uint32_t)(s1 - s0));
                }
                HIPCHK(hipGetLastError());
                times_.add("h2d_pieces_x1", (double)C);
                if (defer_p1_ && batches_.empty()) {
                    HIPCHK(hipMemcpyAsync(mbox64() + MB_P1, ctl_.p + 8, 16, hipMemcpyDeviceToHost, stream_));
                    t.stop_later("partition_with_upload", pending_timers_);
                    p1_ = P1Pending{true, d_bases, d_seg_off, n_seg, n_bases, cap};
                    return finish_partition(n_slices, err);
                }
                t.mark();
                unsigned long long h[2];
                HIPCHK(hipMemcpyAsync(h, ctl_.p + 8, sizeof h, hipMemcpyDeviceToHost, stream_));
                WAIT_STREAM();
                const uint32_t *fl = (const uint32_t *)&h[0];
                if (fl[1]) { err = "a read segment exceeds 32768 bases (split it on the host)"; return -1; }
                if ((uint32_t)h[1] <= cap) {
                    times_.add("partition_with_upload", t.elapsed());
                    if (int rc = finish_partition(n_slices, err)) return rc;
                    return 0;
                }
                times_.add("partition_retry", t.elapsed());
                cap = (uint64_t)(uint32_t)h[1] + 8;
                continue;
            }
            launch_partition_all(wblk, d_bases, d_seg_off, n_seg);
            HIPCHK(hipGetLastError());
            if (defer_p1_ && attempt == 0 && batches_.empty() && piece_list_.empty()) {
                HIPCHK(hipMemcpyAsync(mbox64() + MB_P1, ctl_.p + 8, 16, hipMemcpyDeviceToHost, stream_));
                t.stop_later("partition_kernel", pending_timers_);
                p1_ = P1Pending{true, d_bases, d_seg_off, n_seg, n_bases, cap};
                return finish_partition(n_slices, err);
            }
            t.mark();
            unsigned long long h[2];
            HIPCHK(hipMemcpyAsync(h, ctl_.p + 8, sizeof h, hipMemcpyDeviceToHost, stream_));
            WAIT_STREAM();
            const double ms = t.elapsed();
            const uint32_t *fl = (const uint32_t *)&h[0];
            if (fl[1]) { err = "a read segment exceeds 32768 bases (split it on the host)"; return -1; }
            const uint32_t max_fill = (uint32_t)h[1];
            if (max_fill <= cap) {
                times_.add("partition_kernel", ms);
                if (int rc = finish_partition(n_slices, err)) return rc;
                return 0;
            }
            times_.add("partition_retry", ms);
            cap = (uint64_t)max_fill + 8;
        }
        err = "partition slices overflowed twice";
        return -6;
    }

    int finish_partition(uint64_t n_slices, std::string &err) {
        constexpr int RW = 2 * W;
        have_parts_ = true;
        if (int rc = run_off_.alloc(n_slices, err)) return rc;
        if (int rc = run_cnt_.alloc(n_slices, err)) return rc;
        hipLaunchKernelGGL(k_make_runs, dim3(grid_for(n_slices)), dim3(256), 0, stream_, fill_.p, pp_, recs_.p,
                           (uint32_t)RW, run_off_.p, run_cnt_.p);
        HIPCHK(hipGetLastError());
        run_view_.run_addr16 = run_off_.p; run_view_.run_cnt = run_cnt_.p;
        run_view_.S = pp_.G; run_view_.k = k_; n_count_parts_ = pp_.P;
        return 0;
    }

    struct BatchRecs { DevBuf<uint64_t> dense; std::vector<unsigned long long> part_off;  };

    int pack_current_batch(std::string &err) {
        constexpr int RW = 2 * W;
        DevBuf<unsigned long long> tot, base;
        if (int rc = tot.alloc(pp_.P, err)) return rc;
        if (int rc = base.alloc(pp_.P, err)) return rc;
        hipLaunchKernelGGL(k_part_totals, dim3(pp_.P), dim3(256), 0, stream_, fill_.p, pp_, tot.p);
        HIPCHK(hipGetLastError());
        std::vector<unsigned long long> h(pp_.P);
        HIPCHK(hipMemcpyAsync(h.data(), tot.p, (size_t)pp_.P * 8, hipMemcpyDeviceToHost, stream_));
        WAIT_STREAM();
        std::unique_ptr<BatchRecs> b(new BatchRecs());
        b->part_off.assign(pp_.P + 1, 0);
        for (uint32_t p = 0; p < pp_.P; p++) b->part_off[p + 1] = b->part_off[p] + h[p];
        if (int rc = b->dense.alloc(b->part_off[pp_.P] * RW + 2, err)) return rc;
        HIPCHK(hipMemcpyAsync(base.p, b->part_off.data(), (size_t)pp_.P * 8, hipMemcpyHostToDevice, stream_));
        EvTimer t(stream_, stage_timers_);
        hipLaunchKernelGGL((k_pack_partition<2 * W>), dim3(pp_.P), dim3(256), 0, stream_, recs_.p, fill_.p, pp_, base.p, b->dense.p);
        HIPCHK(hipGetLastError());
        if (t.on()) times_.add("batch_pack_kernel", t.stop());
        WAIT_STREAM();
        batches_.push_back(std::move(b));
        recs_.release(); fill_.release(); run_off_.release(); run_cnt_.release(); have_parts_ = false;
        if (batches_.size() >= env_u64("SHK_MERGE_BATCHES_AT", 192)) return merge_batches(err);
        return 0;
    }

    int merge_batches(std::string &err) {
// ... 15 lines not shown
        hipLaunchKernelGGL((k_merge_runs<RW>), dim3(pp_.P), dim3(256), 0, stream_, run_view_, base.p, m->dense.p);
        HIPCHK(hipGetLastError());
        if (t.on()) times_.add("batch_merge_kernel", t.stop());
        WAIT_STREAM();
        batches_.clear();
        batches_.push_back(std::move(m));
        run_off_.release(); run_cnt_.release(); have_parts_ = false;
        return 0;
    }

    int make_batch_run_view(std::string &err) {
        const uint32_t nb = (uint32_t)batches_.size();
        if (nb > 256) { err = "more than 256 batches per handle"; return -1; }
        const uint64_t n_runs = (uint64_t)pp_.P * nb;
        std::vector<unsigned long long> addr16(n_runs); std::vector<uint32_t> cnt(n_runs);
        for (uint32_t p = 0; p < pp_.P; p++) {
            unsigned long long r = 0;
            for (uint32_t b = 0; b < nb; b++) r += batches_[b]->part_off[p + 1] - batches_[b]->part_off[p];
            if (r > 0xFFFFFFF0ull) { err = "a partition holds more than 2^32 records"; return -1; }
        }
        for (uint32_t p = 0; p < pp_.P; p++)
            for (uint32_t b = 0; b < nb; b++) {
                const BatchRecs &B = *batches_[b];
                const unsigned long long c = B.part_off[p + 1] - B.part_off[p];
                if (c > 0xFFFFFFFFull) { err = "partition too large in one batch"; return -1; }
                addr16[(uint64_t)p * nb + b] = ((unsigned long long)(uintptr_t)B.dense.p >> 4) + B.part_off[p] * (unsigned long long)W;
                cnt[(uint64_t)p * nb + b] = (uint32_t)c;
            }
        if (int rc = run_off_.alloc(n_runs, err)) return rc;
        if (int rc = run_cnt_.alloc(n_runs, err)) return rc;
        HIPCHK(hipMemcpyAsync(run_off_.p, addr16.data(), n_runs * 8, hipMemcpyHostToDevice, stream_));
        HIPCHK(hipMemcpyAsync(run_cnt_.p, cnt.data(), n_runs * 4, hipMemcpyHostToDevice, stream_));
        WAIT_STREAM();
        run_view_.run_addr16 = run_off_.p; run_view_.run_cnt = run_cnt_.p;
        run_view_.S = nb; run_view_.k = k_; n_count_parts_ = pp_.P;
        have_parts_ = true;
        return 0;
    }
    void set_bloom(bool on) override { bloom_ = on; }
    void set_verbose(bool on) override { if (on) { stage_timers_ = true; keep_stages_ = true; } }
    void single_batch_resident(bool on) override { defer_p1_ = on && !global_mode_; }
    void expect_more_batches() override { if (!forced_P_ && batches_.empty() && !have_parts_) forced_P_ = (uint32_t)PART_MAX_P; }

    int run_count_partitions(const RunView &rv, uint32_t n_parts, uint32_t threshold, DevBuf<uint64_t> (&keys)[W],
                             DevBuf<uint32_t> &cnt, uint64_t &n_rows, uint64_t hist_out[500], uint64_t &inst_out,
                             uint64_t cap_hint, double &ms_out, std::string &err) {
        if (n_parts == 0) { n_rows = 0; inst_out = 0; memset(hist_out, 0, 500 * 8); ms_out = 0; return 0; }
        constexpr uint32_t S = CountShared<W>::S;
        const bool repartition = env_u64("SHK_NO_REPARTITION", 0) == 0 && rv.weights == nullptr;
        DevBuf<unsigned long long> dh;
        DevBuf<OvfRec> d_ovf; DevBuf<OvfItem> d_items; DevBuf<uint32_t> d_fill, d_list, d_maxfill, d_new; DevBuf<uint64_t> d_kmers; DevBuf<BucketRef> d_blist; DevBuf<unsigned long long> d_sumfill;
        const bool bloom = bloom_ && !bloom_off_once_;
        unsigned long long bloom_new = 0, bloom_kmer_bytes = 0, bloom_kmer_bytes_exact = 0;
        if (int rc = dh.alloc(500, err)) return rc;
        if (repartition) if (int rc = d_ovf.alloc(n_parts, err)) return rc;
        const bool split = W <= 2 && repartition && !bloom && rv.weights == nullptr && split_ready_ && split_base_.size() == n_parts && split_total_ > 0 &&
                           env_u64("SHK_COUNT_SPLIT", 1) != 0;
        struct DropSplit { Pipeline<W> *me; bool on; ~DropSplit() { if (on) me->shard_drop_dedup(); } } drop_split{this, split};
        uint64_t cap = cap_hint;
        for (int attempt = 0; attempt < (bloom ? 4 : 2); attempt++) {
            bloom_new = 0; bloom_kmer_bytes = 0; bloom_kmer_bytes_exact = 0;
            for (int j = 0; j < W; j++) if (int rc = keys[j].alloc(cap, err)) return rc;
            if (int rc = cnt.alloc(cap, err)) return rc;
            HIPCHK(fill2_async(dh.p, 500 * 8, 0u, ctl_.p, CTL_WORDS * sizeof(unsigned long long), 0u, stream_));
            KeyArr<W> ok; for (int j = 0; j < W; j++) ok.w[j] = keys[j].p;
            const uint32_t probe_parts = (uint32_t)env_u64("SHK_PROBE_PARTS", 512);
            const uint32_t n_probe = (repartition && probe_parts && n_parts / 4 >= probe_parts) ? probe_parts : 0u;
            EvTimer t(stream_);
            if (split) {
                if (int rc = dd_base_.alloc(n_parts, err)) return rc;
                if (int rc = dd_n_.alloc(n_parts, err)) return rc;
                if (int rc = dd_recs_.alloc(split_total_ * 2 * W + 2, err)) return rc;
                if (int rc = dd_w_.alloc(split_total_ + 2, err)) return rc;
                if (split_stride_) {
                    hipLaunchKernelGGL(k_stride_fill, dim3((n_parts + 255) / 256), dim3(256), 0, stream_, dd_base_.p, n_parts, split_stride_);
                    HIPCHK(hipGetLastError());
                } else HIPCHK(hipMemcpyAsync(dd_base_.p, split_base_.data(), (size_t)n_parts * 8, hipMemcpyHostToDevice, stream_));
                const uint32_t defer_after = n_probe / 8;
                EvTimer t_a(stream_, stage_timers_);
                hipLaunchKernelGGL(k_dedupe_partitions<W>, dim3(std::min<uint32_t>(n_parts, 2u * (uint32_t)n_cus_)), dim3(COUNT_THREADS), 0, stream_,
                                   rv, 0u, n_parts, dd_base_.p, dd_recs_.p, dd_w_.p, dd_n_.p, (uint32_t *)(ctl_.p + 12),
                                   d_ovf.p, (uint32_t *)(ctl_.p + 3), defer_after, (S / 10) * 9, (uint32_t *)(ctl_.p + 14) + 1);
                HIPCHK(hipGetLastError());
                if (attempt == 0) t_a.stop_later("count_dedupe_kernel", pending_timers_);
                const uint32_t per_cu = 2u;
                uint32_t merge = (uint32_t)std::min<uint64_t>(std::max<uint64_t>(env_u64("SHK_COUNT_MERGE", 1), 1), 4);
                if (merge == 3) merge = 2;
                while (merge > 1 && (n_parts % merge != 0 || (n_parts / merge) % 256u != 0 || n_parts / merge < 2u * per_cu * (uint32_t)n_cus_)) merge >>= 1;
                const uint32_t n_groups = (n_parts + merge - 1) / merge;
                EmitRanges er{};
                er_groups_ = 0;
                if (n_parts % merge == 0 && (n_groups & (n_groups - 1u)) == 0 && n_groups <= GP_MAX && cap < (1ull << 28) &&
                    env_u64("SHK_GRAPH_RANGES", 1) != 0) {
                    if (int rc = er_off_.alloc(n_groups, err)) return rc;
                    if (int rc = er_msk_.alloc(n_groups, err)) return rc;
                    if (int rc = er_start_.alloc(n_groups, err)) return rc;
                    if (int rc = er_cnt_.alloc(n_groups, err)) return rc;
                    er.tab_cursor = ctl_.p + CTL_ER; er.broken = (uint32_t *)(ctl_.p + CTL_ER + 1);
                    er.off = er_off_.p; er.msk = er_msk_.p; er.start = er_start_.p; er.cnt = er_cnt_.p;
                    er_groups_ = n_groups;
                }
                hipLaunchKernelGGL(k_count_weighted<W>, dim3(std::min<uint32_t>(n_groups, per_cu * (uint32_t)n_cus_)), dim3(COUNT_THREADS), 0, stream_,
                                   dd_recs_.p, dd_w_.p, dd_base_.p, dd_n_.p, 0u, n_parts, merge, rv.k, threshold, dh.p, ok, cnt.p, (unsigned long long)cap,
                                   ctl_.p + 0, ctl_.p + 1, d_ovf.p, (uint32_t *)(ctl_.p + 3), ctl_.p + 14, 0u, defer_after, er);
            } else {
                auto kern = rv.weights ? k_count_partitions<W, true> : k_count_partitions<W, false>;
                hipLaunchKernelGGL(kern, dim3(std::min<uint32_t>(n_parts, (uint32_t)n_cus_)), dim3(COUNT_THREADS), 0, stream_, rv, n_parts, threshold,
                                   dh.p, ok, cnt.p, (unsigned long long)cap, ctl_.p + 0, ctl_.p + 1,
                                   (uint32_t *)(ctl_.p + 2), (const uint32_t *)nullptr, repartition ? d_ovf.p : (OvfRec *)nullptr,
                                   (uint32_t *)(ctl_.p + 3), (uint32_t *)(ctl_.p + 11), n_probe / 2, n_probe / 8);
            }
            HIPCHK(hipGetLastError());
            t.mark();
            unsigned long long h[4], her[2] = {0, 0};
            HIPCHK(hipMemcpyAsync(h, ctl_.p, sizeof h, hipMemcpyDeviceToHost, stream_));
            HIPCHK(hipMemcpyAsync(hist_out, dh.p, 500 * 8, hipMemcpyDeviceToHost, stream_));
            if (split && er_groups_) HIPCHK(hipMemcpyAsync(her, ctl_.p + CTL_ER, sizeof her, hipMemcpyDeviceToHost, stream_));
            WAIT_STREAM();
            ms_out = t.elapsed();
            const uint32_t n_ovf = (uint32_t)h[3];
            if (env_u64("SHK_VERBOSE_TALLY", 0)) fprintf(stderr, "[shk] pass 2: %u partitions, %u handed over, tally tried %u / over %u, split %d\n", n_parts, n_ovf,
                                                    (unsigned)((h[3] >> 32) & 0xFFFFu), (unsigned)(h[3] >> 48), (int)split);
            rows_scattered_ = (uint64_t)n_ovf * 4u > n_parts;
            if (n_ovf) {
                EvTimer t2(stream_);
                std::vector<OvfRec> ov(n_ovf);
                HIPCHK(hipMemcpy(ov.data(), d_ovf.p, (size_t)n_ovf * sizeof(OvfRec), hipMemcpyDeviceToHost));
                std::vector<OvfItem> items;
                items.reserve(n_ovf);
                std::vector<uint32_t> bad;
                uint32_t n_untried = 0;
                const unsigned long long fill_pct = env_u64("SHK_OVF_FILL_PCT", 110), cap_pct = env_u64("SHK_OVF_CAP_PCT", bloom ? 100 : 150);
                for (uint32_t i = 0; i < n_ovf; i++) {
                    if (ov[i].instances >= 0xFFFFFFF0ull) { bad.push_back(ov[i].p); continue; }
                    items.emplace_back();
                    OvfItem &item = items.back();
                    const unsigned long long per = (unsigned long long)S * fill_pct / 100;
                    const uint32_t F = (uint32_t)std::min<unsigned long long>(std::max<unsigned long long>((ov[i].instances + per - 1) / per, 2ull), OVF_MAX_F);
                    if (ov[i].est_distinct == 0) n_untried++;
                    const unsigned long long capb = ov[i].instances * cap_pct / (100ull * F) + 256;
                    item.p = ov[i].p; item.F = F; item.cap = (uint32_t)std::min<unsigned long long>(capb, 0xFFFFFFF0ull);
                    item.pad = 0; item.base = 0;
                }
                size_t n_good_total = 0;
                const int max_passes = (int)env_u64("SHK_OVF_MAX_PASSES", 4);
                for (int pass = 0; pass < max_passes && !items.empty(); pass++) {
// ... 92 lines not shown
            cap = bloom ? n_rows + n_rows / 16 + 4096 : n_rows;
        }
        err = "row buffer overflowed twice";
        return -6;
    }

    int histogram(uint64_t histo[500], uint32_t emit_threshold, std::string &err) override {
        er_ok_ = false;
        if (!global_mode_) {
            memset(histo, 0, 500 * 8);
            n_distinct_ = 0; n_emitted_ = 0; emit_threshold_ = emit_threshold;
            if (!batches_.empty()) {
                if (have_parts_ && recs_.p) if (int rc = pack_current_batch(err)) return rc;
                if (int rc = make_batch_run_view(err)) return rc;
            }
            if (have_parts_) {
                const uint64_t inst_ub_rows = total_rows_hint();
                double ms = 0; uint64_t inst = 0;
                split_base_.assign(n_count_parts_, 0); split_total_ = 0; split_stride_ = 0;
                if (batches_.empty()) {
                    split_stride_ = (unsigned long long)pp_.G * pp_.slice_cap;
                    for (uint32_t p = 0; p < n_count_parts_; p++) split_base_[p] = (unsigned long long)p * pp_.G * pp_.slice_cap;
                    split_total_ = (unsigned long long)n_count_parts_ * pp_.G * pp_.slice_cap;
                } else {
                    for (uint32_t p = 0; p < n_count_parts_; p++) {
                        split_base_[p] = split_total_;
                        for (auto &b : batches_) split_total_ += b->part_off[p + 1] - b->part_off[p];
                    }
                }
                split_ready_ = true;
                int rc_p2 = run_count_partitions(run_view_, n_count_parts_, emit_threshold, ekeys_, ecnt_, n_emitted_, histo, inst,
                                                 inst_ub_rows, ms, err);
                if (p1_.on) {
                    if (rc_p2) { std::string e2; (void)e2; (void)hipStreamSynchronize(stream_); }
                    p1_.on = false;
                    const unsigned long long *h = mbox64() + MB_P1;
                    const uint32_t *fl = (const uint32_t *)&h[0];
                    if (fl[1]) { split_ready_ = false; err = "a read segment exceeds 32768 bases (split it on the host)"; return -1; }
                    if ((uint32_t)h[1] > p1_.cap) {
                        times_.add("partition_retry", 1.0);
                        cap_override_ = (uint64_t)(uint32_t)h[1] + 8;
                        have_parts_ = false; split_ready_ = false;
                        const bool d = defer_p1_; defer_p1_ = false;
                        const int rc1 = count_batch_impl(p1_.d_bases, p1_.d_seg_off, nullptr, nullptr, p1_.n_seg, p1_.n_bases, err);
                        defer_p1_ = d;
                        if (rc1) return rc1;
                        return histogram(histo, emit_threshold, err);
                    }
                }
                if (rc_p2) { split_ready_ = false; return rc_p2; }
                split_ready_ = false;
                times_.add("count_kernel", ms);
                total_instances_ = inst;
            }
            for (int i = 0; i < 500; i++) { histo_[i] = histo[i]; n_distinct_ += histo[i]; }
            return 0;
        }
        DevBuf<unsigned long long> dh;
        if (int rc = dh.alloc(500, err)) return rc;
        HIPCHK(hipMemsetAsync(dh.p, 0, 500 * 8, stream_));
        if (tslots_) {
            EvTimer t(stream_, stage_timers_);
            hipLaunchKernelGGL(k_histogram<W>, dim3(grid_for(tslots_)), dim3(256), 0, stream_, table_view(),
                               tslots_, dh.p);
            HIPCHK(hipGetLastError());
            if (t.on()) times_.add("histogram_kernel", t.stop());
// ... 121 lines not shown
    }
    uint32_t rec_words() const override { return 2 * W; }

    int shard_pack(void *d_send, const uint64_t *base_records, uint32_t n_partitions, std::string &err) override {
        if (!have_parts_) return 0;
        if (n_partitions != pp_.P) { err = "partition count mismatch"; return -1; }
        DevBuf<unsigned long long> base;
        if (int rc = base.alloc(pp_.P, err)) return rc;
        HIPCHK(hipMemcpyAsync(base.p, base_records, (size_t)pp_.P * 8, hipMemcpyHostToDevice, stream_));
        EvTimer t(stream_, stage_timers_);
        hipLaunchKernelGGL((k_pack_partition<2 * W>), dim3(pp_.P), dim3(256), 0, stream_, recs_.p, fill_.p, pp_, base.p,
                           (uint64_t *)d_send);
        HIPCHK(hipGetLastError());
        if (t.on()) times_.add("shard_pack_kernel", t.stop());
        WAIT_STREAM();
        recs_.release(); fill_.release(); run_off_.release(); run_cnt_.release(); have_parts_ = false;
        return 0;
    }

    int shard_dedupe(std::vector<uint64_t> &part_records, std::string &err) override {
        if (!have_parts_) return 0;
        if (part_records.size() < pp_.P) { err = "partition count mismatch"; return -1; }
        std::vector<unsigned long long> base(pp_.P);
        unsigned long long n_raw = 0;
        for (uint32_t p = 0; p < pp_.P; p++) { base[p] = n_raw; n_raw += part_records[p]; }
        if (int rc = dd_base_.alloc(pp_.P, err)) return rc;
        if (int rc = dd_n_.alloc(pp_.P, err)) return rc;
        if (int rc = dd_recs_.alloc(n_raw * 2 * W + 2, err)) return rc;
        if (int rc = dd_w_.alloc(n_raw + 2, err)) return rc;
        HIPCHK(hipMemcpyAsync(dd_base_.p, base.data(), (size_t)pp_.P * 8, hipMemcpyHostToDevice, stream_));
        HIPCHK(fill2_async(ctl_.p + 12, 8, 0u, nullptr, 0, 0u, stream_));
        EvTimer t(stream_, stage_timers_);
        hipLaunchKernelGGL(k_dedupe_partitions<W>, dim3(std::min<uint32_t>(pp_.P, (W <= 2 ? 2u : 1u) * (uint32_t)n_cus_)), dim3(COUNT_THREADS), 0, stream_,
                           run_view_, 0u, pp_.P, dd_base_.p, dd_recs_.p, dd_w_.p, dd_n_.p, (uint32_t *)(ctl_.p + 12),
                           (OvfRec *)nullptr, (uint32_t *)nullptr, 0u, 0u, (uint32_t *)nullptr);
        HIPCHK(hipGetLastError());
        t.mark();
        std::vector<uint32_t> h(pp_.P);
        HIPCHK(hipMemcpyAsync(h.data(), dd_n_.p, (size_t)pp_.P * 4, hipMemcpyDeviceToHost, stream_));
        WAIT_STREAM();
        times_.add("shard_dedupe_kernel", t.elapsed());
        unsigned long long n_dd = 0;
        for (uint32_t p = 0; p < pp_.P; p++) { part_records[p] = h[p]; n_dd += h[p]; }
        times_.add("shard_dedupe_records_in_x1e-6", (double)n_raw * 1e-6);
        times_.add("shard_dedupe_records_out_x1e-6", (double)n_dd * 1e-6);
        have_dedup_ = true;
        return 0;
    }
    void shard_drop_dedup() override { dd_recs_.release(); dd_w_.release(); dd_base_.release(); dd_n_.release(); have_dedup_ = false; }
    int shard_pack_dedup(void *d_send, void *d_send_w, const uint64_t *base_records, uint32_t n_partitions, std::string &err) override {
        if (!have_dedup_) return 0;
        if (n_partitions != pp_.P) { err = "partition count mismatch"; return -1; }
        DevBuf<unsigned long long> base;
        if (int rc = base.alloc(pp_.P, err)) return rc;
        HIPCHK(hipMemcpyAsync(base.p, base_records, (size_t)pp_.P * 8, hipMemcpyHostToDevice, stream_));
        EvTimer t(stream_, stage_timers_);
        hipLaunchKernelGGL((k_pack_dedup<2 * W>), dim3(pp_.P), dim3(256), 0, stream_, dd_recs_.p, dd_w_.p, dd_base_.p, dd_n_.p, base.p,
                           (uint64_t *)d_send, (uint32_t *)d_send_w);
        HIPCHK(hipGetLastError());
        if (t.on()) times_.add("shard_pack_kernel", t.stop());
        WAIT_STREAM();
        shard_drop_dedup();
        recs_.release(); fill_.release(); run_off_.release(); run_cnt_.release(); have_parts_ = false;
        return 0;
    }

    int shard_count(const void *d_recv, const void *d_recv_w, const uint64_t *run_off, const uint32_t *run_cnt, uint32_t n_owned,
                    uint32_t n_sources, uint32_t emit_threshold, uint64_t histo[500], std::string &err) override {
        if (n_sources < 1 || n_sources > 256) { err = "1..256 sources"; return -1; }
        const uint64_t n_runs = (uint64_t)n_owned * n_sources;
        if (int rc = run_off_.alloc(n_runs, err)) return rc;
        if (int rc = run_cnt_.alloc(n_runs, err)) return rc;
        std::vector<unsigned long long> addr16(n_runs);
        for (uint64_t i = 0; i < n_runs; i++) addr16[i] = ((unsigned long long)(uintptr_t)d_recv >> 4) + run_off[i] * (unsigned long long)W;
        if (n_runs) {
            HIPCHK(hipMemcpyAsync(run_off_.p, addr16.data(), n_runs * 8, hipMemcpyHostToDevice, stream_));
            HIPCHK(hipMemcpyAsync(run_cnt_.p, run_cnt, n_runs * 4, hipMemcpyHostToDevice, stream_));
        }
        shard_recv_ = d_recv;
        run_view_.run_addr16 = run_off_.p; run_view_.run_cnt = run_cnt_.p;
        run_view_.S = n_sources; run_view_.k = k_; n_count_parts_ = n_owned;
        run_view_.weights = (const uint32_t *)d_recv_w; run_view_.rec_base16 = (unsigned long long)(uintptr_t)d_recv >> 4;
        uint64_t total_recs = 0;
        for (uint32_t j = 0; j < n_owned; j++) {
            uint64_t r = 0;
            for (uint32_t s = 0; s < n_sources; s++) r += run_cnt[(uint64_t)j * n_sources + s];
            if (r > 0xFFFFFFF0ull) { err = "a partition holds more than 2^32 records"; return -1; }
            total_recs += r;
        }
        memset(histo, 0, 500 * 8);
        n_emitted_ = 0; emit_threshold_ = emit_threshold; n_distinct_ = 0;
        double ms = 0; uint64_t inst = 0;
        have_parts_ = n_runs != 0;
        const uint64_t rows_hint = d_recv_w ? 2 * total_recs + (1u << 16) : std::max<uint64_t>(1u << 16, total_recs);
        if (int rc = run_count_partitions(run_view_, n_owned, emit_threshold, ekeys_, ecnt_, n_emitted_, histo, inst,
                                          rows_hint, ms, err)) return rc;
        times_.add("count_kernel", ms);
        total_instances_ = inst;
        for (int i = 0; i < 500; i++) { histo_[i] = histo[i]; n_distinct_ += histo[i]; }
        return 0;
    }

    int shard_rows(uint32_t threshold, const void **keys_soa, const void **cnt, uint64_t *n, std::string &err) override {
        if (int rc = filter(threshold, err)) return rc;
        for (int j = 0; j < W; j++) keys_soa[j] = skeys_[j].p;
        *cnt = scnt_.p; *n = n_solid_;
        return 0;
    }

    int shard_set_solid(const void *const *keys_soa, const void *cnt, uint64_t n, const uint64_t histo[500],
                        uint64_t total_instances, std::string &err) override {
        if (n >= 0x7FFFFFFFull) { err = "too many solid k-mers for 32-bit node ids"; return -1; }
        DevBuf<uint64_t> nk[W]; DevBuf<uint32_t> nc;
// ... 154 lines not shown
    }

    int check_graph_flags(std::string &err) {
        if (!graph_check_pending_) return 0;
        graph_check_pending_ = false;
        const unsigned long long *h = mbox64() + MB_CTL;
        if ((uint32_t)h[1] == 2u) { err = "graph partition: a row lies outside its counting group's minimiser range"; return -6; }
        if ((uint32_t)h[1] || h[2] > gt_slots_) { err = "graph table overflow"; return -6; }
        return 0;
    }
    int read_ctl(unsigned int &v, int slot, std::string &err) {
        unsigned long long h = 0;
        HIPCHK(hipMemcpyAsync(&h, ctl_.p + slot, 8, hipMemcpyDeviceToHost, stream_));
        WAIT_STREAM();
        v = (unsigned int)h;
        return 0;
    }

    int apply_marks(Graph<W> &g, DevBuf<uint8_t> &mark, DevBuf<uint32_t> &removed, int slot, std::string &err) {
        const uint32_t n = (uint32_t)n_solid_;
        hipLaunchKernelGGL(k_collect_marked, dim3(grid_for(n)), dim3(256), 0, stream_, n, mark.p, alive_.p,
                           removed.p, (unsigned int *)(ctl_.p + slot));
        hipLaunchKernelGGL(k_apply_removed<W>, dim3(1024), dim3(256), 0, stream_, g, removed.p,
                           (const unsigned int *)(ctl_.p + slot));
        HIPCHK(hipGetLastError());
        return 0;
    }

    int correct(bool tips, bool bubbles, std::string &err) override {
        if (!graph_ready_) { err = "graph not built"; return -2; }
        const uint32_t n = (uint32_t)n_solid_;
        tips_removed_ = bubbles_removed_ = 0; rounds_ = 0;
        corr_pending_ = false; corr_tips_ = tips; corr_bubbles_ = bubbles;
        if (n == 0 || (!tips && !bubbles)) return 0;
        if (int rc = corr_.cand.alloc(2ull * n, err)) return rc;
        if (int rc = corr_.removed.alloc(n, err)) return rc;
        if (int rc = corr_.mark.alloc(n, err)) return rc;
        if (!tips) HIPCHK(hipMemsetAsync(corr_.mark.p, 0, n, stream_));
        if (tips) {
            if (int rc = corr_.tip_head.alloc(2ull * n, err)) return rc;
            if (int rc = corr_.tiprec.alloc(2ull * n, err)) return rc;
            if (int rc = corr_.kill.alloc(2ull * n, err)) return rc;
        }
        EvTimer t(stream_, stage_timers_);
        if (int rc = correction_round(0, err)) return rc;
        t.stop_later("correct_total", pending_timers_);
        corr_pending_ = true;
        return 0;
    }
    struct CorrScratch { DevBuf<uint32_t> cand, tip_head, removed; DevBuf<uint8_t> mark, kill; DevBuf<TipRec> tiprec;
                         void release() { cand.release(); tip_head.release(); removed.release(); mark.release(); kill.release(); tiprec.release(); } };
    int correction_round(int round, std::string &err) {
        const uint32_t n = (uint32_t)n_solid_;
        Graph<W> g = graph_view();
        const dim3 G(1024), B(256);
        const bool tips = corr_tips_, bubbles = corr_bubbles_;
        const int s_tip = round == 0 ? 16 : 5, s_bub = round == 0 ? 17 : 6;
        HIPCHK(fill2_async(ctl_.p + 3, 4 * 8, 0u, nullptr, 0, 0u, stream_));
        if (tips) {
            hipLaunchKernelGGL(k_tip_candidates<W>, dim3(grid_for(n)), B, 0, stream_, g, alive_.p,
                               corr_.cand.p, (unsigned int *)(ctl_.p + 3), round == 0 ? (uint2 *)corr_.tip_head.p : (uint2 *)nullptr,
                               round == 0 ? corr_.mark.p : (uint8_t *)nullptr);
            hipLaunchKernelGGL(k_tip_walk<W>, G, B, 0, stream_, g, corr_.cand.p, (const unsigned int *)(ctl_.p + 3),
                               corr_.tiprec.p, (unsigned int *)(ctl_.p + 4), corr_.tip_head.p);
            hipLaunchKernelGGL(k_tip_decide<W>, G, B, 0, stream_, g, corr_.tiprec.p, (const unsigned int *)(ctl_.p + 4),
                               corr_.tip_head.p, corr_.kill.p);
            hipLaunchKernelGGL(k_tip_remove<W>, G, B, 0, stream_, g, corr_.tiprec.p, (const unsigned int *)(ctl_.p + 4),
                               corr_.kill.p, corr_.tip_head.p, corr_.mark.p);
            hipLaunchKernelGGL(k_tip_reset_heads, G, B, 0, stream_, corr_.tiprec.p, (const unsigned int *)(ctl_.p + 4),
                               corr_.tip_head.p);
            HIPCHK(hipGetLastError());
            if (int rc = apply_marks(g, corr_.mark, corr_.removed, s_tip, err)) return rc;
        }
        if (bubbles) {
            HIPCHK(fill2_async(ctl_.p + 3, 8, 0u, nullptr, 0, 0u, stream_));
            hipLaunchKernelGGL(k_fork_candidates<W>, dim3(grid_for(n)), B, 0, stream_, g, alive_.p,
                               corr_.cand.p, (unsigned int *)(ctl_.p + 3));
            hipLaunchKernelGGL(k_bubble<W>, G, B, 0, stream_, g, corr_.cand.p, (const unsigned int *)(ctl_.p + 3), corr_.mark.p);
            HIPCHK(hipGetLastError());
            if (int rc = apply_marks(g, corr_.mark, corr_.removed, s_bub, err)) return rc;
        }
// ... 38 lines not shown
        DevBuf<RingMin> ringmin;
        std::vector<HeadRec> heads;
        uint32_t seg_cap = 0;
        unsigned int n_heads = 0;
        bool heads_on_host = true;
    };
    struct EmitPlan { EmitRec *d_off; char *d_out; char *h_out; uint32_t max_heads; unsigned long long out_cap; bool planned; unsigned long long out_bytes; uint32_t n_emit; };
    int rank_chains(ChainState &cs, bool rings, std::string &err, uint32_t keep_on_device_from = 0xFFFFFFFFu, EmitPlan *plan = nullptr) {
        const uint32_t n = (uint32_t)n_solid_;
        const uint32_t total = 2 * n;
        Graph<W> g = graph_view();
        if (plan) plan->planned = false;
        const bool stage_log = getenv("SHK_STAGE_LOG") != nullptr;
        auto stage = [&](const char *what) {
            if (!stage_log) return;
            const hipError_t e = hipStreamSynchronize(stream_);
            fprintf(stderr, "[rank_chains n=%u] %s done%s\n", n, what, e == hipSuccess ? "" : " (stream error)"); fflush(stderr);
        };
        if (int rc = cs.winfo.alloc(total, err)) return rc;
        if (int rc = cs.frag.alloc(total, err)) return rc;
        if (int rc = cs.spl.alloc(total, err)) return rc;
        if (int rc = cs.ol.alloc(total, err)) return rc;
        const uint32_t split_mask = (1u << (uint32_t)env_u64("SHK_SPLIT_LOG", SPLIT_LOG_DEFAULT)) - 1u;
        const uint32_t tile_rows = (uint32_t)std::min<uint64_t>(std::max<uint64_t>(env_u64("SHK_TILE_ROWS", LF_ROWS), 1), LF_TILE / 2u);
        const int lf_grid = (int)((n + tile_rows - 1) / tile_rows);
        const uint64_t cap_all = std::min<uint64_t>((uint64_t)total + 1024u, 0xFFFFFFF0ull);
        uint64_t seg_cap64 = std::min<uint64_t>(cap_all, env_u64("SHK_SEG_CAP", (uint64_t)total / 12u + 65536u));
        constexpr unsigned int HEADS_SPEC = 512;
        static_assert(MB_MISC * 8 + HEADS_SPEC * sizeof(HeadRec) <= MBOX_BYTES, "mailbox");
        std::vector<HeadRec> &heads = cs.heads;
        unsigned long long hc[4] = {0, 0, 0, 0};
        uint32_t seg_cap = 0;
        EvTimer tr(stream_, stage_timers_);
        for (int attempt = 0;; attempt++) {
            if (attempt > 3) { err = "collapse: the chain ranking did not settle"; return -6; }
            seg_cap = (uint32_t)seg_cap64;
            cs.seg_cap = seg_cap;
            if (int rc = cs.segs.alloc(seg_cap, err)) return rc;
            if (int rc = cs.Ra.alloc(seg_cap, err)) return rc;
            if (int rc = cs.Rb.alloc(seg_cap, err)) return rc;
            if (int rc = cs.slot_of.alloc(seg_cap, err)) return rc;
            if (int rc = cs.fin.alloc(seg_cap, err)) return rc;
            if (int rc = cs.d_heads.alloc(seg_cap, err)) return rc;
            if (int rc = cs.ringmin.alloc(seg_cap, err)) return rc;
            const unsigned long long *skip = corr_pending_ ? ctl_.p + 16 : (const unsigned long long *)nullptr;
            HIPCHK(fill2_async(ctl_.p + 5, 6 * 8, 0u, cs.slot_of.p, (size_t)seg_cap * 4, 0xFFFFFFFFu, stream_));
            unsigned int *d_nspl = (unsigned int *)(ctl_.p + 5);
            uint32_t *d_flags = (uint32_t *)(ctl_.p + 8);
            hipLaunchKernelGGL(k_succ_split<W>, dim3((total + 256 * SS_ITEMS - 1) / (256 * SS_ITEMS)), dim3(256), 0, stream_, g,
                               alive_.p, cs.winfo.p, cs.spl.p, cs.ol.p, d_nspl, split_mask, ctl_.p + 9, skip);
            stage("k_succ_split");
            hipLaunchKernelGGL(k_local_frag<W>, dim3(lf_grid), dim3(LF_THREADS), 0, stream_, n, row_starts_.p, tile_rows, alive_.p, cs.winfo.p, cs.ol.p, cs.frag.p, split_mask, skip,
                               d_nspl, seg_cap, d_flags);
            stage("k_local_frag");
            hipLaunchKernelGGL(k_walk_frags<W>, dim3(grid_for((uint64_t)total / 64u + 16384u, 256, 1 << 20)), dim3(256), 0, stream_,
                               cs.spl.p, (const unsigned int *)d_nspl, cs.frag.p, cs.segs.p, split_mask, ctl_.p + 10, total, d_flags);
            stage("k_walk_frags");
            hipLaunchKernelGGL(k_orphan_cycles<W>, dim3(grid_for(total)), dim3(256), 0, stream_, g, alive_.p, cs.winfo.p, cs.ol.p,
                               cs.frag.p, cs.spl.p, cs.segs.p, d_nspl, seg_cap, d_flags, ctl_.p + 9, ctl_.p + 10);
            HIPCHK(hipGetLastError());
            stage("k_orphan_cycles");
            const int gr = grid_for((uint64_t)total / 64u + 65536u);
            int rounds = 1; { uint64_t reach = RANK_HOPS; while (reach < (uint64_t)seg_cap + 1u) { reach *= RANK_HOPS; rounds++; } }
            hipLaunchKernelGGL(k_rank_init, dim3(gr), dim3(256), 0, stream_, cs.segs.p, (const unsigned int *)d_nspl, cs.Ra.p);
            RankRec *Ri = cs.Ra.p, *Ro = cs.Rb.p;
            for (int r = 0; r < rounds; r++) {
                hipLaunchKernelGGL(k_rank_jump, dim3(gr), dim3(256), 0, stream_, (const unsigned int *)d_nspl, Ri, Ro, (uint32_t)r);
                std::swap(Ri, Ro);
            }
            stage("k_rank_jump");
            const unsigned int *d_ncyc = (const unsigned int *)(ctl_.p + 7);
            hipLaunchKernelGGL(k_rank_tails<W>, dim3(gr), dim3(256), 0, stream_, g, cs.segs.p, (const unsigned int *)d_nspl, Ri, cs.d_heads.p, cs.slot_of.p, cs.ringmin.p,
                               (unsigned int *)(ctl_.p + 6), (unsigned int *)(ctl_.p + 7));
            hipLaunchKernelGGL(k_rank_fin, dim3(gr), dim3(256), 0, stream_, cs.segs.p, (const unsigned int *)d_nspl, Ri, cs.slot_of.p, cs.fin.p);
            stage("k_rank_tails + k_rank_fin");
            hipLaunchKernelGGL(k_tile_final, dim3(lf_grid), dim3(LF_THREADS), 0, stream_, n, row_starts_.p, tile_rows, cs.ol.p, cs.frag.p, cs.fin.p, skip, (const uint32_t *)d_flags);
            stage("k_tile_final");
            if (rings) {
                hipLaunchKernelGGL(k_ring_min1<W>, dim3(1024), dim3(256), 0, stream_, g, alive_.p, cs.ol.p, cs.ringmin.p, d_ncyc);
                hipLaunchKernelGGL(k_ring_min2<W>, dim3(1024), dim3(256), 0, stream_, g, alive_.p, cs.ol.p, cs.ringmin.p, d_ncyc);
                hipLaunchKernelGGL(k_ring_rot<W>, dim3(gr), dim3(256), 0, stream_, g, cs.d_heads.p, (const unsigned int *)(ctl_.p + 6), cs.ringmin.p,
                                   cs.winfo.p, cs.ol.p, d_ncyc, d_flags);
            }
            if (plan) {
                HIPCHK(fill2_async(ctl_.p + 18, 3 * 8, 0u, nullptr, 0, 0u, stream_));
                hipLaunchKernelGGL(k_plan_emit, dim3(1), dim3(1024), 0, stream_, cs.d_heads.p, (const unsigned int *)(ctl_.p + 6), (uint32_t)k_, plan->max_heads,
                                   plan->out_cap, (const uint32_t *)d_flags, plan->d_off, ctl_.p + 18);
                hipLaunchKernelGGL(k_emit<W>, dim3(grid_for(n)), dim3(256), 0, stream_, g, alive_.p, cs.ol.p, plan->d_off, plan->d_out, (const unsigned long long *)(ctl_.p + 18));
                hipLaunchKernelGGL(k_text_to_host_planned, dim3(64), dim3(256), 0, stream_, plan->d_out, plan->h_out, (const unsigned long long *)(ctl_.p + 18));
            }
            HIPCHK(hipGetLastError());
            heads.assign(HEADS_SPEC, HeadRec());
            HIPCHK(hipMemcpyAsync(mbox64() + MB_CTL, ctl_.p, CTL_WORDS * 8, hipMemcpyDeviceToHost, stream_));
            HIPCHK(hipMemcpyAsync(mbox64() + MB_MISC, cs.d_heads.p, (size_t)std::min<uint32_t>(HEADS_SPEC, seg_cap) * sizeof(HeadRec), hipMemcpyDeviceToHost, stream_));
            WAIT_STREAM();
            const unsigned long long *hc0 = mbox64() + MB_CTL;
            if (int rc = check_graph_flags(err)) return rc;
            if (corr_pending_) {
                const unsigned int r1 = (unsigned int)hc0[16], r2 = (unsigned int)hc0[17];
                if (int rc = finish_correction(r1, r2, err)) return rc;
                if (r1 + r2 != 0) continue;
            }
            memcpy(hc, hc0 + 5, sizeof hc);
            const uint32_t flag = (uint32_t)hc[3];
            if ((flag == 4 || flag == 2) && seg_cap64 < cap_all) {
                times_.add("collapse_seg_cap_retry_x1", 1.0);
                seg_cap64 = cap_all;
                continue;
            }
            memcpy(heads.data(), mbox64() + MB_MISC, (size_t)std::min<uint32_t>(HEADS_SPEC, seg_cap) * sizeof(HeadRec));
            if (plan && hc0[18] == 1ull) { plan->planned = true; plan->out_bytes = hc0[19]; plan->n_emit = (uint32_t)hc0[20]; }
            break;
        }
        if ((uint32_t)hc[3]) { err = (uint32_t)hc[3] == 2 ? "collapse: too many short circular unitigs" : ((uint32_t)hc[3] == 3 ? "collapse: ring without a smallest k-mer" : "collapse: broken cycle"); return -6; }
        times_.add("collapse_n_splitters_x1e-3", (double)(unsigned int)hc[0] * 1e-3);
        times_.add("collapse_cycle_splitters_x1e-3", (double)(unsigned int)hc[2] * 1e-3);
        const unsigned int n_heads = (unsigned int)hc[1];
        if (tr.on()) times_.add("collapse_rank_device", tr.stop());
        cs.n_heads = n_heads;
        if (!rings || n_heads >= keep_on_device_from) { heads.resize(std::min<unsigned int>(n_heads, HEADS_SPEC)); cs.heads_on_host = false; return 0; }
        heads.resize(n_heads);
        cs.heads_on_host = true;
        if (n_heads > HEADS_SPEC)
            HIPCHK(hipMemcpy(heads.data() + HEADS_SPEC, cs.d_heads.p + HEADS_SPEC, (size_t)(n_heads - HEADS_SPEC) * sizeof(HeadRec), hipMemcpyDeviceToHost));
        return 0;
    }

    int collapse(std::vector<RawContig> &out, std::string &err, const char **json, size_t *json_len, uint64_t *n_contigs, TextArrival **arrival) override {
        out.clear();
        if (json) *json = nullptr;
        if (arrival) *arrival = nullptr;
        if (!graph_ready_) { err = "graph not built"; return -2; }
        const uint32_t n = (uint32_t)n_solid_;
// ... 670 lines not shown
                hipLaunchKernelGGL(k_text_unpack2, dim3(grid_for(text_w32)), dim3(256), 0, stream_, d_pack.p, text_w32, d_text.p);
                HIPCHK(hipGetLastError());
                times_.add("shard_graph_text_allreduce_MB", (double)(text_w32 * 4) / 1e6);
            }
            HIPCHK(hipMemcpyAsync(hout_.p, d_text.p, text_bytes, hipMemcpyDeviceToHost, stream_));
        }
        stage("6 emission kernels");
        WAIT_STREAM();
        if (te.on()) times_.add("shard_graph_emit", te.stop());
        out.reserve(res.contigs.size());
        for (size_t i = 0; i < res.contigs.size(); i++) {
            RawContig rcg; rcg.kc = res.contigs[i].kc;
            rcg.ext = hout_.p + c_off[i]; rcg.ext_n = res.contigs[i].len_nodes + (uint64_t)(k_ - 1);
            out.push_back(std::move(rcg));
        }
        times_.add("shard_assemble_host_clock", now_ms_() - t_all0);
        return 0;
    }
    template <typename F> static void host_par_ranges(size_t n, F &&fn) {
        const unsigned hw = std::thread::hardware_concurrency();
        const unsigned T = n < 262144 ? 1u : std::min(16u, std::max(1u, hw));
        if (T == 1) { fn((size_t)0, n); return; }
        std::vector<std::thread> ts;
        for (unsigned t = 1; t < T; t++) ts.emplace_back([&fn, n, t, T] { fn(n * t / T, n * (t + 1) / T); });
        fn((size_t)0, n / T);
        for (auto &t : ts) t.join();
    }
    static double now_ms_() { return std::chrono::duration<double, std::milli>(std::chrono::steady_clock::now().time_since_epoch()).count(); }

private:
    int k_;
    hipStream_t stream_ = nullptr; int stream_dev_ = 0;
    hipStream_t copy_stream_ = nullptr;
    ShardComm *wd_comm_ = nullptr;
    bool sh_agreed_ = false;
    StageTimes times_;
    std::vector<EvTimer::Pending> pending_timers_;
    int n_cus_ = 256;
    DevBuf<unsigned long long> ctl_;
    PinnedBuf mbox_;
    unsigned long long *mbox64() { return (unsigned long long *)mbox_.p; }
    static constexpr size_t MBOX_BYTES = 32768;
    static constexpr int MB_P1 = 0 , MB_CTL = 8 , MB_MISC = 64;
    struct P1Pending { bool on; const uint32_t *d_bases, *d_seg_off; uint64_t n_seg, n_bases, cap; };
    P1Pending p1_{false, nullptr, nullptr, 0, 0, 0};
    uint64_t n_host_waits_ = 0;
    bool stage_timers_ = env_u64("SHK_STAGE_TIMERS", 0) != 0;
    bool keep_stages_ = env_u64("SHK_KEEP_STAGES", 0) != 0;
    bool graph_check_pending_ = false, corr_pending_ = false, corr_tips_ = false, corr_bubbles_ = false;
    CorrScratch corr_;
    bool defer_p1_ = false;
    uint64_t cap_override_ = 0;
    DevBuf<uint64_t> tkeys_[W]; DevBuf<uint32_t> tcnt_, tstate_; uint64_t tslots_ = 0;
    struct Batch { const uint32_t *bases, *seg_off; uint64_t n_seg; };
    std::vector<Batch> pending_;
    std::vector<DevPiece> piece_list_;
    uint64_t total_instances_ = 0, n_distinct_ = 0, n_solid_ = 0;
    uint64_t histo_[500] = {0};
    bool global_mode_ = env_u64("SHK_COUNT_MODE_GLOBAL", 0) != 0;
    bool bloom_ = false, bloom_off_once_ = false;
    bool have_parts_ = false;
    bool have_dedup_ = false;
    bool split_ready_ = false;
    std::vector<unsigned long long> split_base_; unsigned long long split_total_ = 0, split_stride_ = 0;
    DevBuf<uint64_t> dd_recs_; DevBuf<uint32_t> dd_w_, dd_n_; DevBuf<unsigned long long> dd_base_;
    PartParams pp_{};
    DevBuf<uint64_t> recs_; DevBuf<uint32_t> fill_;
    DevBuf<unsigned long long> run_off_; DevBuf<uint32_t> run_cnt_;
    RunView run_view_{}; uint32_t n_count_parts_ = 0; uint32_t forced_P_ = 0;
    std::vector<std::unique_ptr<BatchRecs>> batches_;
    const void *shard_recv_ = nullptr;
    DevBuf<uint64_t> ekeys_[W]; DevBuf<uint32_t> ecnt_;
    uint64_t n_emitted_ = 0; uint32_t emit_threshold_ = 0;
    bool rows_scattered_ = false;
    DevBuf<unsigned long long> er_off_; DevBuf<uint32_t> er_msk_, er_start_, er_cnt_;
    uint32_t er_groups_ = 0; uint64_t er_rows_ = 0; bool er_ok_ = false;
    DevBuf<uint64_t> skeys_[W]; DevBuf<uint32_t> scnt_;
    DevBuf<uint64_t> gt_; DevBuf<uint8_t> gt_occ_; DevBuf<uint2> gt_scan_; uint64_t gt_slots_ = 0; uint32_t gp_ = 64;
    DevBuf<unsigned long long> gt_off_; DevBuf<uint32_t> gt_msk_;
    DevBuf<uint8_t> adj_, adj0_, alive_;
    DevBuf<uint32_t> row_starts_;
    PinnedBuf hout_;
    PinnedBuf hends_, hflags_;
    SlabArrival arrival_;
    DevBuf<char> d_out_keep_; DevBuf<unsigned long long> ends_src_;
    std::vector<unsigned long long> ends_src_host_;
    PinnedBuf hjson_;
    DevBuf<uint32_t> nb_;
    bool graph_ready_ = false;
    uint64_t tips_removed_ = 0, bubbles_removed_ = 0; int rounds_ = 0;
    bool sh_active_ = false;
    uint32_t sh_world_ = 1, sh_rank_ = 0, sh_P_ = 1;
    std::vector<uint64_t> sh_gbase_;
    uint64_t n_solid_global_ = 0;
    uint32_t xq_n_ = 0;
    DevBuf<uint32_t> xq_dest_; DevBuf<uint64_t> xq_pay_; DevBuf<unsigned long long> xq_meta_;
    DevBuf<unsigned long long> rt_row_, rt_all_, rt_cur_;
    std::vector<unsigned long long> rt_cur_host_;
    uint64_t rt_extra_host_ = 0;
};
// ... 125 lines not shown
```

sparrowhawk_amd/csrc/preprocess.cpp:

```cpp
#include "preprocess.h"

#include <stdlib.h>
#include <string.h>
#include <algorithm>
#include <thread>
#include <utility>
#include <vector>

#include "fastq_gpu.h"
#include "inflate_gpu.h"
#include "inflate_mt.h"

namespace shk { bool spectrum_fit(const uint64_t *histo500, uint32_t *out); }

using namespace shk;

uint32_t emit_threshold_of(const shk_handle *h) {
    return h->do_fit ? (h->min_count < 1u ? h->min_count : 1u) : h->min_count;
}

namespace {

const int DECLINED = 1;

// ... 6 lines not shown
    const uint64_t batch_bases = std::min<uint64_t>(std::max<uint64_t>(num(getenv("SHK_BATCH_BASES"), 1ull << 31), 1024), 3ull << 30);
    const BgzfWindowKnob window = bgzf_window_knob(2 * batch_bases);
};

template <typename T, void (*Free)(T &)> struct Owned : T {
    Owned() = default;
    Owned(Owned &&o) noexcept : T(std::move(static_cast<T &>(o))) { static_cast<T &>(o) = T(); }
    Owned &operator=(Owned &&o) noexcept { if (this != &o) { reset(); T::operator=(std::move(o)); static_cast<T &>(o) = T(); } return *this; }
    ~Owned() { reset(); }
    void reset() { Free(*this); }
};
using Text = Owned<GpuText, gpu_text_free>;
using Packed = Owned<GpuPacked, gpu_packed_free>;

struct Span { uint64_t base = 0, total = 0; bool pct = true; };
void post_loop(shk_handle *h, uint64_t reads, const Span &sp, uint64_t bytes) {
    std::string s = "loop:" + std::to_string(reads);
    if (sp.pct) s += ":" + std::to_string(sp.total ? (100 * (sp.base + bytes)) / sp.total : 100);
    h->post_mode(s.c_str());
}
void post_device_progress(shk_handle *h, const GpuPacked &gp, const Span &sp, uint64_t n1 = 0) {
    const uint64_t every = h->progress_every();
    for (size_t j = 0; j < gp.progress_bytes.size(); j++) {
        const bool second = (gp.progress_bytes[j] >> 63) != 0;
        post_loop(h, every * (gp.first_mark + j + 1), sp, (second ? n1 : 0) + (gp.progress_bytes[j] & ~(1ull << 63)));
    }
}

int count_one_batch(shk_handle *h, const uint32_t *d_bases, const uint32_t *d_seg_off, uint64_t n_seg, uint64_t n_bases) {
    std::string err;
    const double t0 = now_ms();
    h->batches_started++;
    int rc = h->pipe->count_batch(d_bases, d_seg_off, n_seg, n_bases, err);
    h->pipe->times().add("preprocess_device_total_host_clock", now_ms() - t0);
    return rc ? fail_rc(h, Rc::Device, rc, err) : SHK_OK;
}
int count_pieces(shk_handle *h, const std::vector<DevPiece> &pcs) {
    std::string err;
    const double t0 = now_ms();
    h->batches_started++;
    const int rc = h->pipe->count_batch_pieces(pcs.data(), pcs.size(), err);
    h->pipe->times().add("preprocess_device_total_host_clock", now_ms() - t0);
    return rc ? fail_rc(h, Rc::Device, rc, err) : SHK_OK;
}

int finish_counting(shk_handle *h) {
    std::string err;
    const double t0 = now_ms();
    h->post_loop_edge("loop:end");
    if (!h->do_bloom && h->chunk_size == 0) h->post("preprocess:bulk:sorting");
    int rc = h->pipe->histogram(h->histo, emit_threshold_of(h), err);
    if (rc) return fail(h, SHK_E_DEVICE, err);
    h->used_min_count = h->min_count; h->fit_ok = false;
    if (h->do_fit) {
        h->post_mode("fitting");
        uint32_t v = 0;
        if (spectrum_fit(h->histo, &v)) { h->used_min_count = v; h->fit_ok = true; }
    }
    h->post_mode("filtering");
    rc = h->pipe->filter(h->used_min_count, err);
    if (rc) return fail_rc(h, Rc::DeviceNoParam, rc, err);
    h->post("preprocess:saving");
    h->pre_json = preprocessing_json(h->pipe->n_solid(), h->histo, h->used_min_count);
    h->pipe->times().add("preprocess_device_total_host_clock", now_ms() - t0);
    h->st = St::Preprocessed;
    h->post("preprocess:end");
    return SHK_OK;
}

int run_counting(shk_handle *h, const uint32_t *d_bases, const uint32_t *d_seg_off, uint64_t n_seg, uint64_t n_bases) {
    h->pipe->single_batch_resident(true);
    int rc = count_one_batch(h, d_bases, d_seg_off, n_seg, n_bases);
    if (!rc) rc = finish_counting(h);
    h->pipe->single_batch_resident(false);
    return rc;
// ... 450 lines not shown
```

Before: 179.2.

## Overlap correction round zero with collapse and derive run views without kernel

Runs the first tip/bubble correction round on a separate stream, joined by events, so it proceeds beside the collapse front-end kernels. Collapse kernels gain skip flags so they exit early when correction changed the graph. The k_make_runs kernel is replaced by computing run addresses and counts on the fly from the fill array. Bubble and tip kernels gain gating and any-killed flags, and a stream pool size query is exposed. This adds concurrency and extra bookkeeping in exchange for a risk of wasted collapse work whenever correction changes the graph.

```diff
diff --git a/include/shk.h b/include/shk.h
--- a/include/shk.h
+++ b/include/shk.h
@@ -122,6 +122,7 @@
                                  const uint64_t *min_pos, int tips, int bubbles);
 
 void shk_release_cached_memory(void);
+int shk_pooled_streams(void);
 
 int shk_measure_stream_read(size_t bytes, int iters, double *gbs);
 
diff --git a/sparrowhawk_amd/_lib.py b/sparrowhawk_amd/_lib.py
--- a/sparrowhawk_amd/_lib.py
+++ b/sparrowhawk_amd/_lib.py
@@ -72,6 +72,7 @@
     "shk_host_unitig_assemble": (_vp, [_u32, _u64, _vp, _vp, _vp, _vp, _vp, _vp, _vp, _vp, _int, _int]),
     "shk_device_unitig_assemble": (_vp, [_u32, _u64, _vp, _vp, _vp, _vp, _vp, _vp, _vp, _vp, _int, _int]),
     "shk_release_cached_memory": (None, []),
+    "shk_pooled_streams": (_int, []),
     "shk_measure_stream_read": (_int, [_sz, _int, C.POINTER(C.c_double)]),
     "shk_version": (_cp, []),
 }
diff --git a/sparrowhawk_amd/csrc/api.cpp b/sparrowhawk_amd/csrc/api.cpp
--- a/sparrowhawk_amd/csrc/api.cpp
+++ b/sparrowhawk_amd/csrc/api.cpp
@@ -49,6 +49,7 @@
 static bool comm_is_live(ShardComm *c) { std::lock_guard<std::mutex> lk(g_live_mu); return live_comms().count(c) != 0; }
 
 void shk_release_cached_memory(void) { device_pool_trim(); big_trim(); }
+int shk_pooled_streams(void) { return stream_pool_size(); }
 int shk_measure_stream_read(size_t bytes, int iters, double *gbs) {
     std::string err;
     const int rc = stream_read_gbs(bytes, iters, gbs, err);
diff --git a/sparrowhawk_amd/csrc/collapse.h b/sparrowhawk_amd/csrc/collapse.h
--- a/sparrowhawk_amd/csrc/collapse.h
+++ b/sparrowhawk_amd/csrc/collapse.h
@@ -221,7 +221,9 @@
 __global__ __launch_bounds__(256) void k_walk_frags(const uint32_t *__restrict__ spl, const unsigned int *__restrict__ n_spl_p,
                                                     FragRec *__restrict__ frag, SegRec *__restrict__ segs,
                                                     uint32_t split_mask, unsigned long long *__restrict__ n_covered ,
-                                                    uint32_t total , uint32_t *__restrict__ flags) {
+                                                    uint32_t total , uint32_t *__restrict__ flags,
+                                                    const unsigned long long *__restrict__ skip = nullptr ) {
+    if (skip && (skip[0] | skip[1])) return;
     unsigned long long my_cov = 0;
     const uint32_t n_spl = *n_spl_p;
     for (uint32_t i = blockIdx.x * blockDim.x + threadIdx.x; i < n_spl; i += gridDim.x * blockDim.x) {
@@ -257,7 +259,9 @@
                                                        unsigned int *__restrict__ n_spl,
                                                        uint32_t seg_cap, uint32_t *__restrict__ flags,
                                                        const unsigned long long *__restrict__ n_alive,
-                                                       const unsigned long long *__restrict__ n_covered) {
+                                                       const unsigned long long *__restrict__ n_covered,
+                                                       const unsigned long long *__restrict__ skip = nullptr ) {
+    if (skip && (skip[0] | skip[1])) return;
     if (*n_alive == *n_covered || flags[0] == 4u) return;
     const uint32_t total = g.n * 2;
     for (uint32_t v = blockIdx.x * blockDim.x + threadIdx.x; v < total; v += gridDim.x * blockDim.x) {
@@ -291,7 +295,9 @@
 
 struct RankRec { uint32_t P, A, m, d; unsigned long long K, dK; };
 __global__ __launch_bounds__(256) void k_rank_init(const SegRec *__restrict__ segs, const unsigned int *__restrict__ n_spl_p,
-                                                   RankRec *__restrict__ R) {
+                                                   RankRec *__restrict__ R,
+                                                   const unsigned long long *__restrict__ skip = nullptr ) {
+    if (skip && (skip[0] | skip[1])) return;
     const uint32_t n_spl = *n_spl_p;
     for (uint32_t s = blockIdx.x * blockDim.x + threadIdx.x; s < n_spl; s += gridDim.x * blockDim.x) {
         const SegRec r = segs[s];
@@ -302,7 +308,9 @@
 }
 static constexpr int RANK_HOPS = 8;
 __global__ __launch_bounds__(256) void k_rank_jump(const unsigned int *__restrict__ n_spl_p,
-                                                   const RankRec *__restrict__ Ri, RankRec *__restrict__ Ro, uint32_t round = 0) {
+                                                   const RankRec *__restrict__ Ri, RankRec *__restrict__ Ro, uint32_t round = 0,
+                                                   const unsigned long long *__restrict__ skip = nullptr ) {
+    if (skip && (skip[0] | skip[1])) return;
     const uint32_t n_spl = *n_spl_p;
     {
         unsigned long long reach = 1; for (uint32_t r = 0; r < round; r++) reach *= RANK_HOPS;
@@ -334,7 +342,9 @@
                                                     const RankRec *__restrict__ R,
                                                     HeadRec *__restrict__ heads, uint32_t *__restrict__ slot_of,
                                                     RingMin *__restrict__ ringmin,
-                                                    unsigned int *__restrict__ n_heads, unsigned int *__restrict__ n_cyc) {
+                                                    unsigned int *__restrict__ n_heads, unsigned int *__restrict__ n_cyc,
+                                                    const unsigned long long *__restrict__ skip = nullptr ) {
+    if (skip && (skip[0] | skip[1])) return;
     __shared__ uint32_t blk_cyc;
     if (threadIdx.x == 0) blk_cyc = 0;
     __syncthreads();
@@ -378,7 +388,9 @@
 }
 __global__ __launch_bounds__(256) void k_rank_fin(const SegRec *__restrict__ segs, const unsigned int *__restrict__ n_spl_p,
                                                   const RankRec *__restrict__ R, const uint32_t *__restrict__ slot_of,
-                                                  FinRec *__restrict__ fin) {
+                                                  FinRec *__restrict__ fin,
+                                                  const unsigned long long *__restrict__ skip = nullptr ) {
+    if (skip && (skip[0] | skip[1])) return;
     const uint32_t n_spl = *n_spl_p;
     for (uint32_t s = blockIdx.x * blockDim.x + threadIdx.x; s < n_spl; s += gridDim.x * blockDim.x) {
         const RankRec me = R[s];
diff --git a/sparrowhawk_amd/csrc/count_part.h b/sparrowhawk_amd/csrc/count_part.h
--- a/sparrowhawk_amd/csrc/count_part.h
+++ b/sparrowhawk_amd/csrc/count_part.h
@@ -637,19 +637,16 @@
     int k;
     const uint32_t *weights = nullptr;
     unsigned long long rec_base16 = 0;
+    const uint32_t *fill = nullptr;
+    unsigned long long base16 = 0;
+    uint32_t slice_cap = 0; unsigned long long addr_step = 0;
+    __host__ __device__ __forceinline__ uint32_t cnt_of(uint64_t i) const { return fill ? (fill[i] < slice_cap ? fill[i] : slice_cap) : run_cnt[i]; }
+    __host__ __device__ __forceinline__ unsigned long long addr16_of(uint64_t i) const { return fill ? base16 + i * addr_step : run_addr16[i]; }
 };
-
-__global__ __launch_bounds__(256) void k_make_runs(const uint32_t *__restrict__ fill, PartParams pp,
-                                                   const uint64_t *recs, uint32_t rec_words,
-                                                   unsigned long long *__restrict__ run_addr16,
-                                                   uint32_t *__restrict__ run_cnt) {
-    const uint64_t n = (uint64_t)pp.P * pp.G;
-    const unsigned long long base16 = (unsigned long long)recs >> 4;
-    for (uint64_t i = (uint64_t)blockIdx.x * blockDim.x + threadIdx.x; i < n; i += (uint64_t)gridDim.x * blockDim.x) {
-        run_addr16[i] = base16 + i * pp.slice_cap * (rec_words / 2u);
-        run_cnt[i] = min(fill[i], pp.slice_cap);
-    }
-}
+struct PartBase {
+    const unsigned long long *tab; unsigned long long stride;
+    __device__ __forceinline__ unsigned long long operator[](uint32_t p) const { return tab ? tab[p] : (unsigned long long)p * stride; }
+};
 
 __global__ __launch_bounds__(256) void k_part_totals(const uint32_t *__restrict__ fill, PartParams pp,
                                                      unsigned long long *__restrict__ totals) {
@@ -708,8 +705,8 @@
         uint32_t run = 0;
         for (uint32_t g0 = 0; g0 < S_runs; g0 += 64) {
             const uint32_t g = g0 + threadIdx.x;
-            const uint32_t f = g < S_runs ? rvw.run_cnt[(uint64_t)p * S_runs + g] : 0u;
-            if (g < S_runs) roff[g] = rvw.run_addr16[(uint64_t)p * S_runs + g];
+            const uint32_t f = g < S_runs ? rvw.cnt_of((uint64_t)p * S_runs + g) : 0u;
+            if (g < S_runs) roff[g] = rvw.addr16_of((uint64_t)p * S_runs + g);
             uint32_t incl = f;
             for (int o = 1; o < 64; o <<= 1) { const uint32_t v = __shfl_up(incl, o); if (lane >= o) incl += v; }
             if (g < S_runs) pre[g] = run + incl - f;
@@ -756,8 +753,8 @@
         cnt = 0; addr = 0;
         if (pi < n_parts && threadIdx.x < S_runs) {
             const uint32_t pp = part_list ? part_list[pi] : pi;
-            cnt = rvw.run_cnt[(uint64_t)pp * S_runs + threadIdx.x];
-            addr = rvw.run_addr16[(uint64_t)pp * S_runs + threadIdx.x];
+            cnt = rvw.cnt_of((uint64_t)pp * S_runs + threadIdx.x);
+            addr = rvw.addr16_of((uint64_t)pp * S_runs + threadIdx.x);
         }
     };
     uint32_t nx_cnt; unsigned long long nx_addr;
@@ -977,7 +974,7 @@
 template <int W>
 __global__ __launch_bounds__(COUNT_THREADS, W <= 2 ? 8 : 4) void k_dedupe_partitions(
                                                                      RunView rvw, uint32_t p_first, uint32_t n_parts,
-                                                                     const unsigned long long *__restrict__ base,
+                                                                     PartBase base,
                                                                      uint64_t *__restrict__ out_recs, uint32_t *__restrict__ out_w,
                                                                      uint32_t *__restrict__ n_out, uint32_t *__restrict__ work_counter,
                                                                      OvfRec *__restrict__ ovf , uint32_t *__restrict__ ovf_n,
@@ -1000,7 +997,7 @@
     for (uint32_t pi = blockIdx.x; pi < n_here; pi = pi_next) {
         const uint32_t p = p_first + pi;
         uint32_t f = 0; unsigned long long addr = 0;
-        if (threadIdx.x < S_runs) { f = rvw.run_cnt[(uint64_t)p * S_runs + threadIdx.x]; addr = rvw.run_addr16[(uint64_t)p * S_runs + threadIdx.x]; }
+        if (threadIdx.x < S_runs) { f = rvw.cnt_of((uint64_t)p * S_runs + threadIdx.x); addr = rvw.addr16_of((uint64_t)p * S_runs + threadIdx.x); }
         forced = forced_sh != 0;
         if (forced) {
             unsigned long long inst = 0;
@@ -1145,7 +1142,7 @@
 
 template <int W>
 __global__ __launch_bounds__(COUNT_THREADS, W <= 2 ? 8 : 4) void k_count_weighted(
-    const uint64_t *__restrict__ recs, const uint32_t *__restrict__ weights, const unsigned long long *__restrict__ base,
+    const uint64_t *__restrict__ recs, const uint32_t *__restrict__ weights, PartBase base,
     const uint32_t *__restrict__ n_recs, uint32_t p_first, uint32_t n_parts, uint32_t merge , int k, uint32_t threshold,
     unsigned long long *__restrict__ histo, KeyArr<W> out_keys, uint32_t *__restrict__ out_cnt,
     unsigned long long out_cap, unsigned long long *__restrict__ out_cursor,
@@ -1351,7 +1348,7 @@
         uint32_t run = 0;
         for (uint32_t g0 = 0; g0 < S_runs; g0 += 64) {
             const uint32_t g = g0 + threadIdx.x;
-            uint32_t f = g < S_runs ? rvw.run_cnt[(uint64_t)p * S_runs + g] : 0u;
+            uint32_t f = g < S_runs ? rvw.cnt_of((uint64_t)p * S_runs + g) : 0u;
             uint32_t incl = f;
             for (int o = 1; o < 64; o <<= 1) { uint32_t v = __shfl_up(incl, o); if (lane >= o) incl += v; }
             if (g < S_runs) pre[g] = run + incl - f;
@@ -1366,7 +1363,7 @@
     for (uint32_t r = threadIdx.x; r < R; r += COUNT_THREADS) {
         uint32_t lo = 0, hi = S_runs;
         while (hi - lo > 1) { const uint32_t mid = (lo + hi) >> 1; if (pre[mid] <= r) lo = mid; else hi = mid; }
-        const uint64_t *src = reinterpret_cast<const uint64_t *>(rvw.run_addr16[(uint64_t)p * S_runs + lo] << 4) + (uint64_t)(r - pre[lo]) * RW;
+        const uint64_t *src = reinterpret_cast<const uint64_t *>(rvw.addr16_of((uint64_t)p * S_runs + lo) << 4) + (uint64_t)(r - pre[lo]) * RW;
         Rec<RW> rec;
 #pragma unroll
         for (int o = 0; o < RW; o += 2) {
diff --git a/sparrowhawk_amd/csrc/graph_part.h b/sparrowhawk_amd/csrc/graph_part.h
--- a/sparrowhawk_amd/csrc/graph_part.h
+++ b/sparrowhawk_amd/csrc/graph_part.h
@@ -658,11 +658,13 @@
 __global__ __launch_bounds__(256) void k_tip_remove(Graph<W> g, const TipRec *__restrict__ tips,
                                                     const unsigned int *__restrict__ n_tips_p, const uint8_t *__restrict__ kill,
                                                     uint32_t *__restrict__ tip_head,
-                                                    uint8_t *__restrict__ mark) {
+                                                    uint8_t *__restrict__ mark,
+                                                    unsigned int *__restrict__ any_killed = nullptr ) {
     const uint32_t n_tips = *n_tips_p;
     for (uint32_t a = blockIdx.x * blockDim.x + threadIdx.x; a < n_tips; a += gridDim.x * blockDim.x) {
         const TipRec me = tips[a];
         if (kill[a]) {
+            if (any_killed) *any_killed = 1u;
             uint32_t cur = me.start;
             for (uint32_t i = 0; i < me.len; i++) {
                 mark[cur >> 1] = 1;
@@ -682,7 +684,9 @@
 template <int W>
 __global__ __launch_bounds__(256) void k_fork_candidates(Graph<W> g, const uint8_t *__restrict__ alive,
                                                          uint32_t *__restrict__ cand,
-                                                         unsigned int *__restrict__ n_cand) {
+                                                         unsigned int *__restrict__ n_cand,
+                                                         const unsigned int *__restrict__ gate = nullptr ) {
+    if (gate && *gate) return;
     const int lane = threadIdx.x & 63;
     const uint32_t stride = gridDim.x * blockDim.x;
     const uint32_t n_round = (g.n + stride - 1) / stride * stride;
@@ -704,7 +708,10 @@
 
 template <int W>
 __global__ __launch_bounds__(256) void k_bubble(Graph<W> g, const uint32_t *__restrict__ cand,
-                                                const unsigned int *__restrict__ n_cand_p, uint8_t *__restrict__ mark) {
+                                                const unsigned int *__restrict__ n_cand_p, uint8_t *__restrict__ mark,
+                                                const unsigned int *__restrict__ gate = nullptr ,
+                                                unsigned int *__restrict__ any_marked = nullptr ) {
+    if (gate && *gate) return;
     const uint32_t T_BUB = 2u * (uint32_t)g.k;
     const uint32_t n_cand = *n_cand_p;
     for (uint32_t c = blockIdx.x * blockDim.x + threadIdx.x; c < n_cand; c += gridDim.x * blockDim.x) {
@@ -759,6 +766,7 @@
                 if (better) best = false;
             }
             if (grp >= 2 && !best) {
+                if (any_marked) *any_marked = 1u;
                 uint32_t cur = first[a];
                 for (uint32_t i = 0; i < len[a]; i++) {
                     mark[cur >> 1] = 1;
diff --git a/sparrowhawk_amd/csrc/pipeline.h b/sparrowhawk_amd/csrc/pipeline.h
--- a/sparrowhawk_amd/csrc/pipeline.h
+++ b/sparrowhawk_amd/csrc/pipeline.h
@@ -78,6 +78,7 @@
     virtual uint64_t n_solid_global() const = 0;
     virtual int shard_assemble(ShardComm *comm, bool tips, bool bubbles, std::vector<RawContig> &out, std::string &err) = 0;
     virtual StageTimes &times() = 0;
+    virtual void add_time(const char *name, double v) = 0;
     virtual void drain() = 0;
     virtual void *stream() = 0;
     virtual int device() const = 0;
@@ -104,6 +105,7 @@
 int device_upload(const void *host, size_t bytes, void **dptr, std::string &err);
 void device_free(void *dptr);
 void device_pool_trim();
+int stream_pool_size();
 void *device_pool_alloc(size_t &bytes);
 int stream_read_gbs(size_t bytes, int iters, double *gbs, std::string &err);
 void device_pool_release(void *p, size_t bytes);
diff --git a/sparrowhawk_amd/csrc/pipeline.hip b/sparrowhawk_amd/csrc/pipeline.hip
--- a/sparrowhawk_amd/csrc/pipeline.hip
+++ b/sparrowhawk_amd/csrc/pipeline.hip
@@ -39,6 +39,7 @@
 
 static constexpr uint32_t NIL = 0xFFFFFFFFu;
 static constexpr int CTL_WORDS = 32;
+static constexpr int CTL_P1 = 26;
 static constexpr int CTL_ER = 22;
 static constexpr uint32_t GP_MAX = 131072;
 static constexpr uint64_t EMPTY64 = ~0ull;
@@ -245,6 +246,8 @@
     (void)hipStreamDestroy(s);
 }
 
+int stream_pool_size() { std::lock_guard<std::mutex> lk(g_stream_mu); return (int)stream_cache().size(); }
+
 static std::mutex &upload_token(int dev) { static std::mutex m[16]; return m[(unsigned)dev % 16u]; }
 
 static inline int grid_for(uint64_t work, int block = 256, int max_blocks = 256 * 16) {
@@ -315,9 +318,6 @@
     for (unsigned long long i = (unsigned long long)blockIdx.x * blockDim.x + threadIdx.x; i < na + nb; i += stride) {
         if (i < na) a[i] = va; else b[i - na] = vb;
     }
-}
-__global__ __launch_bounds__(256) void k_stride_fill(unsigned long long *out, uint32_t n, unsigned long long stride) {
-    for (uint32_t i = blockIdx.x * blockDim.x + threadIdx.x; i < n; i += gridDim.x * blockDim.x) out[i] = (unsigned long long)i * stride;
 }
 static inline hipError_t fill2_async(void *a, size_t bytes_a, uint32_t va, void *b, size_t bytes_b, uint32_t vb, hipStream_t st) {
     const unsigned long long na = bytes_a / 4, nb = bytes_b / 4;
@@ -415,6 +415,9 @@
         drain();
         EvTimer::resolve(pending_timers_, times_);
         if (copy_stream_) { (void)hipStreamSynchronize(copy_stream_); stream_pool_put(stream_dev_ + 1000, copy_stream_); }
+        if (corr_ev_fork_) (void)hipEventDestroy(corr_ev_fork_);
+        if (corr_ev_join_) (void)hipEventDestroy(corr_ev_join_);
+        if (corr_stream_) stream_pool_put(stream_dev_ + 2000, corr_stream_);
         if (stream_) stream_pool_put(stream_dev_, stream_);
     }
     int init(std::string &err) {
@@ -427,8 +430,10 @@
         return 0;
     }
     StageTimes &times() override { EvTimer::resolve(pending_timers_, times_); return times_; }
+    void add_time(const char *name, double v) override { times_.add(name, v); }
     void drain() override {
         if (copy_stream_) (void)hipStreamSynchronize(copy_stream_);
+        corr_join_now();
         if (!stream_) return;
         std::string e;
         if (wd_comm_) (void)comm_stream_wait(wd_comm_, stream_, e);
@@ -495,7 +500,7 @@
     template <int WBLK, int NBLK>
     void launch_partition_t(const uint32_t *d_bases, const uint32_t *d_seg_off, uint32_t n_seg) {
         hipLaunchKernelGGL((k_partition<W, WBLK, NBLK>), dim3(pp_.G), dim3(PART_THREADS), 0, stream_, d_bases, d_seg_off,
-                           n_seg, pp_, recs_.p, fill_.p, (uint32_t *)(ctl_.p + 8));
+                           n_seg, pp_, recs_.p, fill_.p, (uint32_t *)(ctl_.p + CTL_P1));
     }
     void launch_partition(int win, const uint32_t *d_bases, const uint32_t *d_seg_off, uint32_t n_seg) {
         if (win == 20) launch_partition_t<10, 2>(d_bases, d_seg_off, n_seg);
@@ -570,8 +575,10 @@
             pp_.slice_cap = (uint32_t)cap;
             const uint64_t n_slices = (uint64_t)P * pp_.G;
             if (int rc = recs_.alloc(n_slices * cap * RW, err)) return rc;
-            if (int rc = fill_.alloc(n_slices, err)) return rc;
-            HIPCHK(fill2_async(fill_.p, n_slices * 4, 0u, ctl_.p, CTL_WORDS * sizeof(unsigned long long), 0u, stream_));
+            dh_off_ = (n_slices + 1) & ~(uint64_t)1;
+            if (int rc = fill_.alloc(dh_off_ + 2 * 500, err)) return rc;
+            HIPCHK(fill2_async(fill_.p, (dh_off_ + 2 * 500) * 4, 0u, ctl_.p, CTL_WORDS * sizeof(unsigned long long), 0u, stream_));
+            p2_zeroed_ = false; p1_copied_ = false;
             EvTimer t(stream_);
             if (h_bases && attempt == 0) {
                 uint64_t C = env_u64("SHK_H2D_PIECES", 4);
@@ -597,14 +604,14 @@
                 HIPCHK(hipGetLastError());
                 times_.add("h2d_pieces_x1", (double)C);
                 if (defer_p1_ && batches_.empty()) {
-                    HIPCHK(hipMemcpyAsync(mbox64() + MB_P1, ctl_.p + 8, 16, hipMemcpyDeviceToHost, stream_));
                     t.stop_later("partition_with_upload", pending_timers_);
+                    p2_zeroed_ = true;
                     p1_ = P1Pending{true, d_bases, d_seg_off, n_seg, n_bases, cap};
                     return finish_partition(n_slices, err);
                 }
                 t.mark();
                 unsigned long long h[2];
-                HIPCHK(hipMemcpyAsync(h, ctl_.p + 8, sizeof h, hipMemcpyDeviceToHost, stream_));
+                HIPCHK(hipMemcpyAsync(h, ctl_.p + CTL_P1, sizeof h, hipMemcpyDeviceToHost, stream_));
                 WAIT_STREAM();
                 const uint32_t *fl = (const uint32_t *)&h[0];
                 if (fl[1]) { err = "a read segment exceeds 32768 bases (split it on the host)"; return -1; }
@@ -620,14 +627,14 @@
             launch_partition_all(wblk, d_bases, d_seg_off, n_seg);
             HIPCHK(hipGetLastError());
             if (defer_p1_ && attempt == 0 && batches_.empty() && piece_list_.empty()) {
-                HIPCHK(hipMemcpyAsync(mbox64() + MB_P1, ctl_.p + 8, 16, hipMemcpyDeviceToHost, stream_));
                 t.stop_later("partition_kernel", pending_timers_);
+                p2_zeroed_ = true;
                 p1_ = P1Pending{true, d_bases, d_seg_off, n_seg, n_bases, cap};
                 return finish_partition(n_slices, err);
             }
             t.mark();
             unsigned long long h[2];
-            HIPCHK(hipMemcpyAsync(h, ctl_.p + 8, sizeof h, hipMemcpyDeviceToHost, stream_));
+            HIPCHK(hipMemcpyAsync(h, ctl_.p + CTL_P1, sizeof h, hipMemcpyDeviceToHost, stream_));
             WAIT_STREAM();
             const double ms = t.elapsed();
             const uint32_t *fl = (const uint32_t *)&h[0];
@@ -645,15 +652,12 @@
         return -6;
     }
 
-    int finish_partition(uint64_t n_slices, std::string &err) {
-        constexpr int RW = 2 * W;
+    int finish_partition(uint64_t, std::string &) {
         have_parts_ = true;
-        if (int rc = run_off_.alloc(n_slices, err)) return rc;
-        if (int rc = run_cnt_.alloc(n_slices, err)) return rc;
-        hipLaunchKernelGGL(k_make_runs, dim3(grid_for(n_slices)), dim3(256), 0, stream_, fill_.p, pp_, recs_.p,
-                           (uint32_t)RW, run_off_.p, run_cnt_.p);
-        HIPCHK(hipGetLastError());
-        run_view_.run_addr16 = run_off_.p; run_view_.run_cnt = run_cnt_.p;
+        run_off_.release(); run_cnt_.release();
+        run_view_.run_addr16 = nullptr; run_view_.run_cnt = nullptr;
+        run_view_.fill = fill_.p; run_view_.base16 = (unsigned long long)(uintptr_t)recs_.p >> 4;
+        run_view_.slice_cap = pp_.slice_cap; run_view_.addr_step = (unsigned long long)pp_.slice_cap * (unsigned long long)W;
         run_view_.S = pp_.G; run_view_.k = k_; n_count_parts_ = pp_.P;
         return 0;
     }
@@ -735,7 +739,7 @@
         HIPCHK(hipMemcpyAsync(run_off_.p, addr16.data(), n_runs * 8, hipMemcpyHostToDevice, stream_));
         HIPCHK(hipMemcpyAsync(run_cnt_.p, cnt.data(), n_runs * 4, hipMemcpyHostToDevice, stream_));
         WAIT_STREAM();
-        run_view_.run_addr16 = run_off_.p; run_view_.run_cnt = run_cnt_.p;
+        run_view_.run_addr16 = run_off_.p; run_view_.run_cnt = run_cnt_.p; run_view_.fill = nullptr;
         run_view_.S = nb; run_view_.k = k_; n_count_parts_ = pp_.P;
         have_parts_ = true;
         return 0;
@@ -751,11 +755,14 @@
         if (n_parts == 0) { n_rows = 0; inst_out = 0; memset(hist_out, 0, 500 * 8); ms_out = 0; return 0; }
         constexpr uint32_t S = CountShared<W>::S;
         const bool repartition = env_u64("SHK_NO_REPARTITION", 0) == 0 && rv.weights == nullptr;
-        DevBuf<unsigned long long> dh;
+        DevBuf<unsigned long long> dh_own;
+        const bool pre_zeroed = p2_zeroed_ && fill_.p && rv.fill == fill_.p;
+        p2_zeroed_ = false;
         DevBuf<OvfRec> d_ovf; DevBuf<OvfItem> d_items; DevBuf<uint32_t> d_fill, d_list, d_maxfill, d_new; DevBuf<uint64_t> d_kmers; DevBuf<BucketRef> d_blist; DevBuf<unsigned long long> d_sumfill;
         const bool bloom = bloom_ && !bloom_off_once_;
         unsigned long long bloom_new = 0, bloom_kmer_bytes = 0, bloom_kmer_bytes_exact = 0;
-        if (int rc = dh.alloc(500, err)) return rc;
+        if (!pre_zeroed) if (int rc = dh_own.alloc(500, err)) return rc;
+        struct { unsigned long long *p; } dh{pre_zeroed ? (unsigned long long *)(fill_.p + dh_off_) : dh_own.p};
         if (repartition) if (int rc = d_ovf.alloc(n_parts, err)) return rc;
         const bool split = W <= 2 && repartition && !bloom && rv.weights == nullptr && split_ready_ && split_base_.size() == n_parts && split_total_ > 0 &&
                            env_u64("SHK_COUNT_SPLIT", 1) != 0;
@@ -765,24 +772,22 @@
             bloom_new = 0; bloom_kmer_bytes = 0; bloom_kmer_bytes_exact = 0;
             for (int j = 0; j < W; j++) if (int rc = keys[j].alloc(cap, err)) return rc;
             if (int rc = cnt.alloc(cap, err)) return rc;
-            HIPCHK(fill2_async(dh.p, 500 * 8, 0u, ctl_.p, CTL_WORDS * sizeof(unsigned long long), 0u, stream_));
+            if (!(pre_zeroed && attempt == 0)) HIPCHK(fill2_async(dh.p, 500 * 8, 0u, ctl_.p, CTL_P1 * sizeof(unsigned long long), 0u, stream_));
             KeyArr<W> ok; for (int j = 0; j < W; j++) ok.w[j] = keys[j].p;
             const uint32_t probe_parts = (uint32_t)env_u64("SHK_PROBE_PARTS", 512);
             const uint32_t n_probe = (repartition && probe_parts && n_parts / 4 >= probe_parts) ? probe_parts : 0u;
             EvTimer t(stream_);
             if (split) {
-                if (int rc = dd_base_.alloc(n_parts, err)) return rc;
+                if (!split_stride_) if (int rc = dd_base_.alloc(n_parts, err)) return rc;
                 if (int rc = dd_n_.alloc(n_parts, err)) return rc;
                 if (int rc = dd_recs_.alloc(split_total_ * 2 * W + 2, err)) return rc;
                 if (int rc = dd_w_.alloc(split_total_ + 2, err)) return rc;
-                if (split_stride_) {
-                    hipLaunchKernelGGL(k_stride_fill, dim3((n_parts + 255) / 256), dim3(256), 0, stream_, dd_base_.p, n_parts, split_stride_);
-                    HIPCHK(hipGetLastError());
-                } else HIPCHK(hipMemcpyAsync(dd_base_.p, split_base_.data(), (size_t)n_parts * 8, hipMemcpyHostToDevice, stream_));
+                if (!split_stride_) HIPCHK(hipMemcpyAsync(dd_base_.p, split_base_.data(), (size_t)n_parts * 8, hipMemcpyHostToDevice, stream_));
+                const PartBase dd_base{split_stride_ ? (const unsigned long long *)nullptr : dd_base_.p, split_stride_};
                 const uint32_t defer_after = n_probe / 8;
                 EvTimer t_a(stream_, stage_timers_);
                 hipLaunchKernelGGL(k_dedupe_partitions<W>, dim3(std::min<uint32_t>(n_parts, 2u * (uint32_t)n_cus_)), dim3(COUNT_THREADS), 0, stream_,
-                                   rv, 0u, n_parts, dd_base_.p, dd_recs_.p, dd_w_.p, dd_n_.p, (uint32_t *)(ctl_.p + 12),
+                                   rv, 0u, n_parts, dd_base, dd_recs_.p, dd_w_.p, dd_n_.p, (uint32_t *)(ctl_.p + 12),
                                    d_ovf.p, (uint32_t *)(ctl_.p + 3), defer_after, (S / 10) * 9, (uint32_t *)(ctl_.p + 14) + 1);
                 HIPCHK(hipGetLastError());
                 if (attempt == 0) t_a.stop_later("count_dedupe_kernel", pending_timers_);
@@ -804,7 +809,7 @@
                     er_groups_ = n_groups;
                 }
                 hipLaunchKernelGGL(k_count_weighted<W>, dim3(std::min<uint32_t>(n_groups, per_cu * (uint32_t)n_cus_)), dim3(COUNT_THREADS), 0, stream_,
-                                   dd_recs_.p, dd_w_.p, dd_base_.p, dd_n_.p, 0u, n_parts, merge, rv.k, threshold, dh.p, ok, cnt.p, (unsigned long long)cap,
+                                   dd_recs_.p, dd_w_.p, dd_base, dd_n_.p, 0u, n_parts, merge, rv.k, threshold, dh.p, ok, cnt.p, (unsigned long long)cap,
                                    ctl_.p + 0, ctl_.p + 1, d_ovf.p, (uint32_t *)(ctl_.p + 3), ctl_.p + 14, 0u, defer_after, er);
             } else {
                 auto kern = rv.weights ? k_count_partitions<W, true> : k_count_partitions<W, false>;
@@ -815,6 +820,10 @@
             }
             HIPCHK(hipGetLastError());
             t.mark();
+            if (p1_.on && !p1_copied_) {
+                HIPCHK(hipMemcpyAsync(mbox64() + MB_P1, ctl_.p + CTL_P1, 16, hipMemcpyDeviceToHost, stream_));
+                p1_copied_ = true;
+            }
             unsigned long long h[4], her[2] = {0, 0};
             HIPCHK(hipMemcpyAsync(h, ctl_.p, sizeof h, hipMemcpyDeviceToHost, stream_));
             HIPCHK(hipMemcpyAsync(hist_out, dh.p, 500 * 8, hipMemcpyDeviceToHost, stream_));
@@ -973,6 +982,11 @@
                 int rc_p2 = run_count_partitions(run_view_, n_count_parts_, emit_threshold, ekeys_, ecnt_, n_emitted_, histo, inst,
                                                  inst_ub_rows, ms, err);
                 if (p1_.on) {
+                    if (!p1_copied_) {
+                        (void)hipMemcpyAsync(mbox64() + MB_P1, ctl_.p + CTL_P1, 16, hipMemcpyDeviceToHost, stream_);
+                        (void)hipStreamSynchronize(stream_);
+                        p1_copied_ = true;
+                    }
                     if (rc_p2) { std::string e2; (void)e2; (void)hipStreamSynchronize(stream_); }
                     p1_.on = false;
                     const unsigned long long *h = mbox64() + MB_P1;
@@ -1160,7 +1174,7 @@
         HIPCHK(fill2_async(ctl_.p + 12, 8, 0u, nullptr, 0, 0u, stream_));
         EvTimer t(stream_, stage_timers_);
         hipLaunchKernelGGL(k_dedupe_partitions<W>, dim3(std::min<uint32_t>(pp_.P, (W <= 2 ? 2u : 1u) * (uint32_t)n_cus_)), dim3(COUNT_THREADS), 0, stream_,
-                           run_view_, 0u, pp_.P, dd_base_.p, dd_recs_.p, dd_w_.p, dd_n_.p, (uint32_t *)(ctl_.p + 12),
+                           run_view_, 0u, pp_.P, PartBase{dd_base_.p, 0ull}, dd_recs_.p, dd_w_.p, dd_n_.p, (uint32_t *)(ctl_.p + 12),
                            (OvfRec *)nullptr, (uint32_t *)nullptr, 0u, 0u, (uint32_t *)nullptr);
         HIPCHK(hipGetLastError());
         t.mark();
@@ -1206,7 +1220,7 @@
             HIPCHK(hipMemcpyAsync(run_cnt_.p, run_cnt, n_runs * 4, hipMemcpyHostToDevice, stream_));
         }
         shard_recv_ = d_recv;
-        run_view_.run_addr16 = run_off_.p; run_view_.run_cnt = run_cnt_.p;
+        run_view_.run_addr16 = run_off_.p; run_view_.run_cnt = run_cnt_.p; run_view_.fill = nullptr;
         run_view_.S = n_sources; run_view_.k = k_; n_count_parts_ = n_owned;
         run_view_.weights = (const uint32_t *)d_recv_w; run_view_.rec_base16 = (unsigned long long)(uintptr_t)d_recv >> 4;
         uint64_t total_recs = 0;
@@ -1427,7 +1441,8 @@
         const uint32_t n = (uint32_t)n_solid_;
         tips_removed_ = bubbles_removed_ = 0; rounds_ = 0;
         corr_pending_ = false; corr_tips_ = tips; corr_bubbles_ = bubbles;
-        if (n == 0 || (!tips && !bubbles)) return 0;
+        corr_overlap_ = false;
+        if (n == 0 || (!tips && !bubbles)) { report_correction(false, false); return 0; }
         if (int rc = corr_.cand.alloc(2ull * n, err)) return rc;
         if (int rc = corr_.removed.alloc(n, err)) return rc;
         if (int rc = corr_.mark.alloc(n, err)) return rc;
@@ -1437,11 +1452,89 @@
             if (int rc = corr_.tiprec.alloc(2ull * n, err)) return rc;
             if (int rc = corr_.kill.alloc(2ull * n, err)) return rc;
         }
+        if (!sh_active_ && env_u64("SHK_CORR_OVERLAP", 1) != 0) {
+            if (int rc = launch_round0_detection(err)) { corr_join_now(); return rc; }
+            corr_overlap_ = true;
+        } else {
+            EvTimer t(stream_, stage_timers_);
+            if (int rc = correction_round(0, err)) return rc;
+            t.stop_later("correct_total", pending_timers_);
+        }
+        corr_pending_ = true;
+        return 0;
+    }
+    void corr_join_now() {
+        if (corr_fork_open_ && corr_stream_) (void)hipStreamSynchronize(corr_stream_);
+        corr_fork_open_ = false;
+    }
+    int launch_round0_detection(std::string &err) {
+        const uint32_t n = (uint32_t)n_solid_;
+        Graph<W> g = graph_view();
+        const dim3 G(1024), B(256);
+        if (!corr_stream_) corr_stream_ = stream_pool_get(stream_dev_ + 2000);
+        if (!corr_stream_) HIPCHK(hipStreamCreateWithFlags(&corr_stream_, hipStreamNonBlocking));
+        if (!corr_ev_fork_) HIPCHK(hipEventCreateWithFlags(&corr_ev_fork_, hipEventDisableTiming));
+        if (!corr_ev_join_) HIPCHK(hipEventCreateWithFlags(&corr_ev_join_, hipEventDisableTiming));
+        hipStream_t s2 = corr_stream_;
+        HIPCHK(hipEventRecord(corr_ev_fork_, stream_));
+        HIPCHK(hipStreamWaitEvent(s2, corr_ev_fork_, 0));
+        corr_fork_open_ = true;
+        EvTimer t(s2, stage_timers_);
+        unsigned int *any_tip = (unsigned int *)(ctl_.p + 16), *any_bub = (unsigned int *)(ctl_.p + 17);
+        HIPCHK(fill2_async(ctl_.p + 3, 2 * 8, 0u, ctl_.p + 15, 3 * 8, 0u, s2));
+        if (corr_tips_) {
+            hipLaunchKernelGGL(k_tip_candidates<W>, dim3(grid_for(n)), B, 0, s2, g, alive_.p,
+                               corr_.cand.p, (unsigned int *)(ctl_.p + 3), (uint2 *)corr_.tip_head.p, corr_.mark.p);
+            hipLaunchKernelGGL(k_tip_walk<W>, G, B, 0, s2, g, corr_.cand.p, (const unsigned int *)(ctl_.p + 3),
+                               corr_.tiprec.p, (unsigned int *)(ctl_.p + 4), corr_.tip_head.p);
+            hipLaunchKernelGGL(k_tip_decide<W>, G, B, 0, s2, g, corr_.tiprec.p, (const unsigned int *)(ctl_.p + 4),
+                               corr_.tip_head.p, corr_.kill.p);
+            hipLaunchKernelGGL(k_tip_remove<W>, G, B, 0, s2, g, corr_.tiprec.p, (const unsigned int *)(ctl_.p + 4),
+                               corr_.kill.p, corr_.tip_head.p, corr_.mark.p, any_tip);
+            hipLaunchKernelGGL(k_tip_reset_heads, G, B, 0, s2, corr_.tiprec.p, (const unsigned int *)(ctl_.p + 4),
+                               corr_.tip_head.p);
+        }
+        if (corr_bubbles_) {
+            hipLaunchKernelGGL(k_fork_candidates<W>, dim3(grid_for(n)), B, 0, s2, g, alive_.p,
+                               corr_.cand.p, (unsigned int *)(ctl_.p + 15), (const unsigned int *)any_tip);
+            hipLaunchKernelGGL(k_bubble<W>, G, B, 0, s2, g, corr_.cand.p, (const unsigned int *)(ctl_.p + 15), corr_.mark.p,
+                               (const unsigned int *)any_tip, any_bub);
+        }
+        HIPCHK(hipGetLastError());
+        t.stop_later("correct_total", pending_timers_);
+        HIPCHK(hipEventRecord(corr_ev_join_, s2));
+        return 0;
+    }
+    int apply_round0(unsigned int f1, unsigned int f2, unsigned int &n1, unsigned int &n2, std::string &err) {
+        n1 = n2 = 0;
+        times_.add("correct_overlap_x1", 1.0);
+        times_.add("correct_round0_applied_x1", (f1 | f2) ? 1.0 : 0.0);
+        times_.add("correct_round0_bubbles_redone_x1", (f1 && corr_bubbles_) ? 1.0 : 0.0);
+        if (!(f1 | f2)) return 0;
+        const uint32_t n = (uint32_t)n_solid_;
+        Graph<W> g = graph_view();
         EvTimer t(stream_, stage_timers_);
-        if (int rc = correction_round(0, err)) return rc;
-        t.stop_later("correct_total", pending_timers_);
-        corr_pending_ = true;
-        return 0;
+        HIPCHK(fill2_async(ctl_.p + 16, 2 * 8, 0u, ctl_.p + 3, 8, 0u, stream_));
+        if (f1) {
+            if (int rc = apply_marks(g, corr_.mark, corr_.removed, 16, err)) return rc;
+            if (corr_bubbles_) {
+                hipLaunchKernelGGL(k_fork_candidates<W>, dim3(grid_for(n)), dim3(256), 0, stream_, g, alive_.p,
+                                   corr_.cand.p, (unsigned int *)(ctl_.p + 3));
+                hipLaunchKernelGGL(k_bubble<W>, dim3(1024), dim3(256), 0, stream_, g, corr_.cand.p, (const unsigned int *)(ctl_.p + 3), corr_.mark.p);
+                HIPCHK(hipGetLastError());
+                if (int rc = apply_marks(g, corr_.mark, corr_.removed, 17, err)) return rc;
+            }
+        } else if (int rc = apply_marks(g, corr_.mark, corr_.removed, 17, err)) return rc;
+        HIPCHK(hipMemcpyAsync(mbox64() + MB_MISC, ctl_.p + 16, 16, hipMemcpyDeviceToHost, stream_));
+        WAIT_STREAM();
+        n1 = (unsigned int)mbox64()[MB_MISC]; n2 = (unsigned int)mbox64()[MB_MISC + 1];
+        if (t.on()) times_.add("correct_total", t.stop());
+        return 0;
+    }
+    void report_correction(bool overlapped, bool applied) {
+        times_.add("correct_tips_removed_x1", (double)tips_removed_);
+        times_.add("correct_bubbles_removed_x1", (double)bubbles_removed_);
+        if (!overlapped) { times_.add("correct_overlap_x1", 0.0); times_.add("correct_round0_applied_x1", applied ? 1.0 : 0.0); }
     }
     struct CorrScratch { DevBuf<uint32_t> cand, tip_head, removed; DevBuf<uint8_t> mark, kill; DevBuf<TipRec> tiprec;
                          void release() { cand.release(); tip_head.release(); removed.release(); mark.release(); kill.release(); tiprec.release(); } };
@@ -1546,6 +1639,7 @@
         unsigned long long hc[4] = {0, 0, 0, 0};
         uint32_t seg_cap = 0;
         EvTimer tr(stream_, stage_timers_);
+        struct JoinOnExit { Pipeline<W> *me; ~JoinOnExit() { me->corr_join_now(); } } join_on_exit{this};
         for (int attempt = 0;; attempt++) {
             if (attempt > 3) { err = "collapse: the chain ranking did not settle"; return -6; }
             seg_cap = (uint32_t)seg_cap64;
@@ -1558,35 +1652,41 @@
             if (int rc = cs.d_heads.alloc(seg_cap, err)) return rc;
             if (int rc = cs.ringmin.alloc(seg_cap, err)) return rc;
             const unsigned long long *skip = corr_pending_ ? ctl_.p + 16 : (const unsigned long long *)nullptr;
+            const bool beside = corr_pending_ && corr_overlap_;
+            const unsigned long long *skip_front = beside ? (const unsigned long long *)nullptr : skip;
             HIPCHK(fill2_async(ctl_.p + 5, 6 * 8, 0u, cs.slot_of.p, (size_t)seg_cap * 4, 0xFFFFFFFFu, stream_));
             unsigned int *d_nspl = (unsigned int *)(ctl_.p + 5);
             uint32_t *d_flags = (uint32_t *)(ctl_.p + 8);
             hipLaunchKernelGGL(k_succ_split<W>, dim3((total + 256 * SS_ITEMS - 1) / (256 * SS_ITEMS)), dim3(256), 0, stream_, g,
-                               alive_.p, cs.winfo.p, cs.spl.p, cs.ol.p, d_nspl, split_mask, ctl_.p + 9, skip);
+                               alive_.p, cs.winfo.p, cs.spl.p, cs.ol.p, d_nspl, split_mask, ctl_.p + 9, skip_front);
             stage("k_succ_split");
-            hipLaunchKernelGGL(k_local_frag<W>, dim3(lf_grid), dim3(LF_THREADS), 0, stream_, n, row_starts_.p, tile_rows, alive_.p, cs.winfo.p, cs.ol.p, cs.frag.p, split_mask, skip,
+            hipLaunchKernelGGL(k_local_frag<W>, dim3(lf_grid), dim3(LF_THREADS), 0, stream_, n, row_starts_.p, tile_rows, alive_.p, cs.winfo.p, cs.ol.p, cs.frag.p, split_mask, skip_front,
                                d_nspl, seg_cap, d_flags);
             stage("k_local_frag");
+            if (beside) {
+                HIPCHK(hipStreamWaitEvent(stream_, corr_ev_join_, 0));
+                stage("correction round 0 joined");
+            }
             hipLaunchKernelGGL(k_walk_frags<W>, dim3(grid_for((uint64_t)total / 64u + 16384u, 256, 1 << 20)), dim3(256), 0, stream_,
-                               cs.spl.p, (const unsigned int *)d_nspl, cs.frag.p, cs.segs.p, split_mask, ctl_.p + 10, total, d_flags);
+                               cs.spl.p, (const unsigned int *)d_nspl, cs.frag.p, cs.segs.p, split_mask, ctl_.p + 10, total, d_flags, skip);
             stage("k_walk_frags");
             hipLaunchKernelGGL(k_orphan_cycles<W>, dim3(grid_for(total)), dim3(256), 0, stream_, g, alive_.p, cs.winfo.p, cs.ol.p,
-                               cs.frag.p, cs.spl.p, cs.segs.p, d_nspl, seg_cap, d_flags, ctl_.p + 9, ctl_.p + 10);
+                               cs.frag.p, cs.spl.p, cs.segs.p, d_nspl, seg_cap, d_flags, ctl_.p + 9, ctl_.p + 10, skip);
             HIPCHK(hipGetLastError());
             stage("k_orphan_cycles");
             const int gr = grid_for((uint64_t)total / 64u + 65536u);
             int rounds = 1; { uint64_t reach = RANK_HOPS; while (reach < (uint64_t)seg_cap + 1u) { reach *= RANK_HOPS; rounds++; } }
-            hipLaunchKernelGGL(k_rank_init, dim3(gr), dim3(256), 0, stream_, cs.segs.p, (const unsigned int *)d_nspl, cs.Ra.p);
+            hipLaunchKernelGGL(k_rank_init, dim3(gr), dim3(256), 0, stream_, cs.segs.p, (const unsigned int *)d_nspl, cs.Ra.p, skip);
             RankRec *Ri = cs.Ra.p, *Ro = cs.Rb.p;
             for (int r = 0; r < rounds; r++) {
-                hipLaunchKernelGGL(k_rank_jump, dim3(gr), dim3(256), 0, stream_, (const unsigned int *)d_nspl, Ri, Ro, (uint32_t)r);
+                hipLaunchKernelGGL(k_rank_jump, dim3(gr), dim3(256), 0, stream_, (const unsigned int *)d_nspl, Ri, Ro, (uint32_t)r, skip);
                 std::swap(Ri, Ro);
             }
             stage("k_rank_jump");
             const unsigned int *d_ncyc = (const unsigned int *)(ctl_.p + 7);
             hipLaunchKernelGGL(k_rank_tails<W>, dim3(gr), dim3(256), 0, stream_, g, cs.segs.p, (const unsigned int *)d_nspl, Ri, cs.d_heads.p, cs.slot_of.p, cs.ringmin.p,
-                               (unsigned int *)(ctl_.p + 6), (unsigned int *)(ctl_.p + 7));
-            hipLaunchKernelGGL(k_rank_fin, dim3(gr), dim3(256), 0, stream_, cs.segs.p, (const unsigned int *)d_nspl, Ri, cs.slot_of.p, cs.fin.p);
+                               (unsigned int *)(ctl_.p + 6), (unsigned int *)(ctl_.p + 7), skip);
+            hipLaunchKernelGGL(k_rank_fin, dim3(gr), dim3(256), 0, stream_, cs.segs.p, (const unsigned int *)d_nspl, Ri, cs.slot_of.p, cs.fin.p, skip);
             stage("k_rank_tails + k_rank_fin");
             hipLaunchKernelGGL(k_tile_final, dim3(lf_grid), dim3(LF_THREADS), 0, stream_, n, row_starts_.p, tile_rows, cs.ol.p, cs.frag.p, cs.fin.p, skip, (const uint32_t *)d_flags);
             stage("k_tile_final");
@@ -1608,11 +1708,19 @@
             HIPCHK(hipMemcpyAsync(mbox64() + MB_CTL, ctl_.p, CTL_WORDS * 8, hipMemcpyDeviceToHost, stream_));
             HIPCHK(hipMemcpyAsync(mbox64() + MB_MISC, cs.d_heads.p, (size_t)std::min<uint32_t>(HEADS_SPEC, seg_cap) * sizeof(HeadRec), hipMemcpyDeviceToHost, stream_));
             WAIT_STREAM();
+            corr_fork_open_ = false;
             const unsigned long long *hc0 = mbox64() + MB_CTL;
             if (int rc = check_graph_flags(err)) return rc;
             if (corr_pending_) {
-                const unsigned int r1 = (unsigned int)hc0[16], r2 = (unsigned int)hc0[17];
+                unsigned int r1 = (unsigned int)hc0[16], r2 = (unsigned int)hc0[17];
+                const bool was_beside = corr_overlap_;
+                if (was_beside) {
+                    corr_overlap_ = false;
+                    const unsigned int f1 = r1, f2 = r2;
+                    if (int rc = apply_round0(f1, f2, r1, r2, err)) return rc;
+                }
                 if (int rc = finish_correction(r1, r2, err)) return rc;
+                report_correction(was_beside, r1 + r2 != 0);
                 if (r1 + r2 != 0) continue;
             }
             memcpy(hc, hc0 + 5, sizeof hc);
@@ -2349,6 +2457,10 @@
     int k_;
     hipStream_t stream_ = nullptr; int stream_dev_ = 0;
     hipStream_t copy_stream_ = nullptr;
+    hipStream_t corr_stream_ = nullptr;
+    hipEvent_t corr_ev_fork_ = nullptr, corr_ev_join_ = nullptr;
+    bool corr_overlap_ = false;
+    bool corr_fork_open_ = false;
     ShardComm *wd_comm_ = nullptr;
     bool sh_agreed_ = false;
     StageTimes times_;
@@ -2383,6 +2495,9 @@
     DevBuf<uint64_t> dd_recs_; DevBuf<uint32_t> dd_w_, dd_n_; DevBuf<unsigned long long> dd_base_;
     PartParams pp_{};
     DevBuf<uint64_t> recs_; DevBuf<uint32_t> fill_;
+    uint64_t dh_off_ = 0;
+    bool p2_zeroed_ = false;
+    bool p1_copied_ = false;
     DevBuf<unsigned long long> run_off_; DevBuf<uint32_t> run_cnt_;
     RunView run_view_{}; uint32_t n_count_parts_ = 0; uint32_t forced_P_ = 0;
     std::vector<std::unique_ptr<BatchRecs>> batches_;
diff --git a/sparrowhawk_amd/csrc/preprocess.cpp b/sparrowhawk_amd/csrc/preprocess.cpp
--- a/sparrowhawk_amd/csrc/preprocess.cpp
+++ b/sparrowhawk_amd/csrc/preprocess.cpp
@@ -62,7 +62,7 @@
     const double t0 = now_ms();
     h->batches_started++;
     int rc = h->pipe->count_batch(d_bases, d_seg_off, n_seg, n_bases, err);
-    h->pipe->times().add("preprocess_device_total_host_clock", now_ms() - t0);
+    h->pipe->add_time("preprocess_device_total_host_clock", now_ms() - t0);
     return rc ? fail_rc(h, Rc::Device, rc, err) : SHK_OK;
 }
 int count_pieces(shk_handle *h, const std::vector<DevPiece> &pcs) {
@@ -70,7 +70,7 @@
     const double t0 = now_ms();
     h->batches_started++;
     const int rc = h->pipe->count_batch_pieces(pcs.data(), pcs.size(), err);
-    h->pipe->times().add("preprocess_device_total_host_clock", now_ms() - t0);
+    h->pipe->add_time("preprocess_device_total_host_clock", now_ms() - t0);
     return rc ? fail_rc(h, Rc::Device, rc, err) : SHK_OK;
 }
 
```

New measurement: 181.0 (median of 5 runs). 1.01x the previous value.
